# karpathy/minbpe

Hardware: AMD Instinct MI355X
Metric: BPE merges/sec (higher is better)
Workload: dtype int32; 1 GPU; regex1g: RegexTokenizer.train, 1 GB synth seed 2, vocab 32000; mode=default, parallelism=single

## Files before the change

### minbpe_amd/_native.py

```python
import ctypes as C
import os
import sys

import numpy as np

_HERE = os.path.dirname(os.path.abspath(__file__))
LIB_PATH = os.environ.get("MINBPE_AMD_LIB", os.path.join(_HERE, "lib", "libbpe_hip.so"))

BPE_OK = 0
BPE_E_HIP = -1
BPE_E_ARG = -2
BPE_E_EMPTY_STATS = -3
BPE_E_STATE = -4
BPE_E_CAP = -5
BPE_E_LIMIT = -6
BPE_E_INTERNAL = -7

PROF_KINDS = ("widen", "pair_count", "argmax", "merge", "table", "encode", "decode")

if not os.path.exists(LIB_PATH):
    raise ImportError(
        f"{LIB_PATH} is missing: build it with `python -m minbpe_amd.build` "
        "(hipcc --offload-arch=gfx950). minbpe_amd has no CPU fallback.")

# ... 387 lines not shown
                return 1

        cb = ALLREDUCE_FN(_cb)
        rc = _lib.bpe_dp_train_cb(self._h, num_merges, rank, nranks, C.cast(cb, C.c_void_p), None, _ptr(pairs),
                                  _ptr(counts), _ptr(lens), C.byref(done))
        d = done.value
        self.last_train = dict(
            pairs=list(map(tuple, pairs[:2 * d].reshape(d, 2).tolist())),
            counts=counts[:d].tolist(), lens=lens[:d].tolist(), iter_ms=None, n_done=d)
        if raised:
            raise raised[0]
        self._check(rc)
        return self.last_train

    def encode_batch(self, pairs, merge_ids, data, offsets=None):
        buf = np.frombuffer(data, dtype=np.uint8) if not isinstance(data, np.ndarray) else data
        off, n_off = self._offsets(offsets)
        n_chunks = n_off if off is not None else 1
        pm = np.ascontiguousarray(pairs, dtype=np.int32).reshape(-1)
        M = len(pm) // 2
        mi = None if merge_ids is None else np.ascontiguousarray(merge_ids, dtype=np.int32)
        out = np.empty(max(len(buf), 1), np.int32)
        oo = np.zeros(n_chunks + 1, np.uint64)
        n_out = _u64(0)
        self._check(_lib.bpe_encode_batch(self._h, _ptr(pm) if M else None, _ptr(mi), M,
                                          _ptr(buf) if len(buf) else None, len(buf), _ptr(off),
                                          n_off, _ptr(out), _ptr(oo), C.byref(n_out)))
        return out[:n_out.value], oo

    def encode_batch_resident(self, pairs, merge_ids, d_bytes: int, n: int, d_offsets: int, n_chunks: int,
                              d_ids_out: int, d_out_offsets: int) -> int:
        p = np.ascontiguousarray(pairs, dtype=np.int32).reshape(-1)
        mids = None if merge_ids is None else np.ascontiguousarray(merge_ids, dtype=np.int32)
        total = _u64(0)
        self._check(_lib.bpe_encode_batch_resident(
            self._h, _ptr(p) if len(p) else None, None if mids is None else _ptr(mids), len(p) // 2,
            C.c_void_p(d_bytes), n, C.c_void_p(d_offsets), n_chunks, C.c_void_p(d_ids_out), C.c_void_p(d_out_offsets),
            C.byref(total)))
        return int(total.value)

    def decode_set_vocab(self, blob: bytes, offsets):
        buf = np.frombuffer(blob, dtype=np.uint8)
        off = np.ascontiguousarray(offsets, dtype=np.uint64)
        self._check(_lib.bpe_decode_set_vocab(self._h, _ptr(buf) if len(buf) else None, _ptr(off),
                                              len(off) - 1))

    def decode_batch(self, ids, doc_offsets=None):
        arr = np.ascontiguousarray(ids, dtype=np.int32)
        nb, bad = _u64(0), _u64(0)
        rc = _lib.bpe_decode_batch(self._h, _ptr(arr) if len(arr) else None, len(arr), C.byref(nb),
                                   C.byref(bad))
        if rc == BPE_E_ARG and bad.value != 0xFFFFFFFFFFFFFFFF:
            raise InvalidToken(int(bad.value))
        self._check(rc)
        out = np.empty(max(nb.value, 1), np.uint8)
        if doc_offsets is None:
            self._check(_lib.bpe_decode_read(self._h, _ptr(out), len(out), None, 0, None))
            return out[:nb.value].tobytes()
        doff = np.ascontiguousarray(doc_offsets, dtype=np.uint64)
        boff = np.zeros(len(doff), np.uint64)
        self._check(_lib.bpe_decode_read(self._h, _ptr(out), len(out), _ptr(doff), len(doff), _ptr(boff)))
        return out[:nb.value].tobytes(), boff

    def decode_set_sparse(self, sparse_ids, v_dense: int):
        arr = np.ascontiguousarray(sparse_ids, dtype=np.int32)
        self._check(_lib.bpe_decode_set_sparse(self._h, _ptr(arr) if len(arr) else None, len(arr), int(v_dense)))

    def decode_batch_resident(self, d_ids: int, id_width: int, n: int, d_doc_off: int, k: int, d_out: int, out_cap: int,
                              d_boff: int) -> int:
        nb, bad = _u64(0), _u64(0)
        rc = _lib.bpe_decode_batch_resident(self._h, C.c_void_p(d_ids), id_width, n, C.c_void_p(d_doc_off), k,
                                            C.c_void_p(d_out), out_cap, C.c_void_p(d_boff), C.byref(nb), C.byref(bad))
        if rc == BPE_E_ARG and bad.value != 0xFFFFFFFFFFFFFFFF:
            raise InvalidToken(int(bad.value))
        if rc == BPE_E_CAP:
            raise OutputTooSmall(int(nb.value), (_lib.bpe_last_error(self._h) or b"").decode())
        self._check(rc)
        return int(nb.value)

    def prof_reset(self):
        self._check(_lib.bpe_prof_reset(self._h))

    def train_stats(self):
        out = np.zeros(11, np.uint64)
        self._check(_lib.bpe_train_stats_ex(self._h, _ptr(out), 11))
        return dict(dense=int(out[0]), sparse=int(out[1]), index_builds=int(out[2]), slots=int(out[3]),
                    lean=int(out[4]), deferred=int(out[5]), chained=int(out[6]), steps=int(out[7]),
                    selections=int(out[8]), slot_ids=int(out[9]), fused_steps=int(out[10]))

    def prof_read(self):
        k = len(PROF_KINDS)
        ms = np.zeros(k, np.float64)
        launches = np.zeros(k, np.uint64)
        nbytes = np.zeros(k, np.uint64)
        self._check(_lib.bpe_prof_read(self._h, _ptr(ms), _ptr(launches), _ptr(nbytes)))
        return {name: dict(ms=float(ms[i]), launches=int(launches[i]), alg_bytes=int(nbytes[i]))
                for i, name in enumerate(PROF_KINDS)}
```

### minbpe_amd/csrc/api/api_basic.hip

```cpp

extern "C" {

const char *bpe_version(void) { return "minbpe_amd libbpe_hip 0.1 (gfx950)"; }

const char *bpe_last_error(bpe_ctx *ctx) { return ctx ? ctx->err.c_str() : g_create_err.c_str(); }

int bpe_create(int device_id, bpe_ctx **out) {
    if (!out) return fail(nullptr, BPE_E_ARG, "out is NULL");
    *out = nullptr;
    int ndev = 0;
    hipError_t e = hipGetDeviceCount(&ndev);
    if (e != hipSuccess || ndev == 0)
        return fail(nullptr, BPE_E_HIP, "no HIP device available: %s",
                    e != hipSuccess ? hipGetErrorString(e) : "device count is 0");
    if (device_id < 0 || device_id >= ndev)
        return fail(nullptr, BPE_E_ARG, "device %d out of range (%d devices)", device_id, ndev);
    bpe_ctx *c = new bpe_ctx();
    c->device = device_id;
    auto bail = [&](const char *what, hipError_t er) {
        int rc = fail(nullptr, BPE_E_HIP, "%s failed: %s", what, hipGetErrorString(er));
        delete c;
        return rc;
    };
    if ((e = hipSetDevice(device_id)) != hipSuccess) return bail("hipSetDevice", e);
// ... 87 lines not shown
    } else if (!strcmp(name, "sparse")) {
        if (value < 0 || value > 2) return fail(c, BPE_E_ARG, "sparse must be 0 (never), 1 (auto) or 2 (always)");
        c->use_sparse = (int)value;
    } else if (!strcmp(name, "rep_max")) {
        if (value < 0 || value > 8) return fail(c, BPE_E_ARG, "rep_max must be 0..8");
        c->rep_max = (int)value;
    } else if (!strcmp(name, "rep_min")) {
        if (value < 0 || value > 8) return fail(c, BPE_E_ARG, "rep_min: 0..8");
        c->rep_min = value;
    } else if (!strcmp(name, "lds_delta")) {
        c->lds_delta = value != 0;
    } else if (!strcmp(name, "exp_no_delta")) {
        c->exp_no_delta = value != 0;
    } else if (!strcmp(name, "tie_window")) {
        c->tie_window = value != 0;
    } else if (!strcmp(name, "tie_index")) {
        c->tie_index = value != 0;
    } else if (!strcmp(name, "sparse_ratio")) {
        if (value < 1 || value > 64) return fail(c, BPE_E_ARG, "sparse_ratio must be 1..64");
        c->sparse_ratio = (int)value;
    } else if (!strcmp(name, "lean")) {
        if (value < 0 || value > 2) return fail(c, BPE_E_ARG, "lean must be 0 (never), 1 (auto) or 2 (always)");
        c->lean = (int)value;
    } else if (!strcmp(name, "lean_backoff")) {
        c->lean_backoff = value != 0;
    } else if (!strcmp(name, "lean_count")) {
        if (value < 0) return fail(c, BPE_E_ARG, "lean_count must be >= 0");
        c->lean_count = value;
    } else if (!strcmp(name, "lean_grid")) {
        if (value < 1 || value > 65535) return fail(c, BPE_E_ARG, "lean_grid must be 1..65535");
        c->lean_grid = (int)value;
    } else if (!strcmp(name, "enc_chain")) {
        c->enc_chain = value != 0;
    } else if (!strcmp(name, "enc_cache")) {
        c->enc_cache = value != 0;
    } else if (!strcmp(name, "enc_hash_bits")) {
        if (value < 0 || value > 40) return fail(c, BPE_E_ARG, "enc_hash_bits must be 0..40");
        c->enc_hash_bits = (int)value;
    } else if (!strcmp(name, "dec_copy")) {
        c->dec_copy = value != 0;
    } else if (!strcmp(name, "dec_window")) {
        if (value < 1024 || value > 32768 || value % 16) return fail(c, BPE_E_ARG, "dec_window: 1024..32768 bytes, a multiple of 16");
        c->dec_window = (int)value;
    } else if (!strcmp(name, "dec_tile")) {
        if (value < 256 || value > 16384 || value % 256) return fail(c, BPE_E_ARG, "dec_tile: 256..16384 tokens, a multiple of 256");
        c->dec_tile = (int)value;
    } else if (!strcmp(name, "prof_stride")) {
        if (value < 1 || value > 1024) return fail(c, BPE_E_ARG, "prof_stride must be 1..1024");
        c->prof_stride = (int)value;
    } else if (!strcmp(name, "lean_select")) {
        c->lean_select = value != 0;
    } else if (!strcmp(name, "aa_sparse")) {
        c->aa_sparse = value != 0;
    } else if (!strcmp(name, "dp_force_comm")) {
        c->dp_force_comm = value != 0;
    } else if (!strcmp(name, "dp_kcap")) {
        if (value < 1 || value > DP_KCAP_MAX) return fail(c, BPE_E_ARG, "dp_kcap must be 1..%d", DP_KCAP_MAX);
        c->dp_kcap = (int)value;
    } else if (!strcmp(name, "fuse_load")) {
        c->fuse_load = value != 0;
    } else if (!strcmp(name, "chain_dense")) {
        c->chain_dense = value != 0;
    } else if (!strcmp(name, "chain_prefetch")) {
        c->chain_prefetch = value != 0;
    } else if (!strcmp(name, "count_is_removed")) {
        c->count_is_removed = value != 0;
    } else if (!strcmp(name, "enc_long")) {
        c->enc_long = value != 0;
    } else if (!strcmp(name, "small_slots")) {
        if (value < 0 || value > 2) return fail(c, BPE_E_ARG, "small_slots: 0, 1 or 2");
        c->small_slots = (int)value;
    } else if (!strcmp(name, "chain_kcap")) {
        if (value < 1 || value > CH_KSWEEP) return fail(c, BPE_E_ARG, "chain_kcap must be 1..%d", CH_KSWEEP);
        c->chain_kcap = (int)value;
    } else if (!strcmp(name, "enc_replay")) {
        if (value < 0 || value > 1) return fail(c, BPE_E_ARG, "enc_replay must be 0 or 1");
        c->enc_replay = (int)value;
    } else if (!strcmp(name, "pinned_upload")) {
        if (value < 0 || value > 1) return fail(c, BPE_E_ARG, "pinned_upload must be 0 or 1");
        c->pinned_upload = (int)value;
    } else if (!strcmp(name, "fuse_step")) {
        if (value < 0 || value > 1) return fail(c, BPE_E_ARG, "fuse_step must be 0 or 1");
        c->fuse_step = (int)value;
    } else if (!strcmp(name, "pool_hint")) {
        if (value < 0 || value > 128) return fail(c, BPE_E_ARG, "pool_hint must be 0..128");
        c->pool_hint = (int)value;
    } else if (!strcmp(name, "chain_scan")) {
        if (value < 1 || value > 255) return fail(c, BPE_E_ARG, "chain_scan must be 1..255");
        c->chain_scan = value;
    } else if (!strcmp(name, "chain")) {
        c->chain = value != 0;
    } else if (!strcmp(name, "lean_chain")) {
        c->lean_chain = value != 0;
    } else if (!strcmp(name, "lean_sum")) {
        c->lean_sum = value != 0;
    } else if (!strcmp(name, "lean_scan")) {
        if (value < 1 || value > 1024) return fail(c, BPE_E_ARG, "lean_scan must be 1..1024");
        c->lean_scan = (int)value;
    } else if (!strcmp(name, "repack_acc")) {
        if (value < 0 || value > 10000) return fail(c, BPE_E_ARG, "repack_acc must be 0..10000");
        c->repack_acc = (int)value;
    } else if (!strcmp(name, "depth")) {
        if (value < 0 || value > 64) return fail(c, BPE_E_ARG, "depth must be 0..64");
        c->depth = (int)value;
    } else {
        return fail(c, BPE_E_ARG, "unknown option '%s'", name);
    }
    return BPE_OK;
}

static int check_offsets(bpe_ctx *c, const uint64_t *chunk_offsets, uint64_t n_chunks, uint64_t n) {
    if (!chunk_offsets) return BPE_OK;
    auto scan = [&](uint64_t lo, uint64_t hi) -> uint64_t {
        uint64_t prev = lo ? chunk_offsets[lo - 1] : 0;
        for (uint64_t i = lo; i < hi; i++) {
            const uint64_t o = chunk_offsets[i];
            if (o < prev || o > n) return i;
            prev = o;
        }
        return ~0ull;
    };
    uint64_t bad = ~0ull;
    const unsigned hw = std::max(1u, std::thread::hardware_concurrency());
    const uint64_t T = n_chunks < (1ull << 22) ? 1 : std::max<uint64_t>(1, std::min<uint64_t>(16, hw / 2));
    if (T == 1) {
        bad = scan(0, n_chunks);
    } else {
        std::vector<uint64_t> first(T, ~0ull);
        std::vector<std::thread> pool;
        const uint64_t per = (n_chunks + T - 1) / T;
        for (uint64_t w = 0; w < T; w++)
            pool.emplace_back([&, w] { first[w] = scan(std::min(n_chunks, w * per), std::min(n_chunks, (w + 1) * per)); });
        for (std::thread &t : pool) t.join();
        for (uint64_t w = 0; w < T; w++) bad = std::min(bad, first[w]);
    }
    if (bad != ~0ull)
        return fail(c, BPE_E_ARG, "chunk_offsets[%llu] = %llu: offsets must ascend and stay <= n = %llu",
                    (unsigned long long)bad, (unsigned long long)chunk_offsets[bad], (unsigned long long)n);
    return BPE_OK;
}

static int load_bytes_impl(bpe_ctx *c, const uint8_t *bytes, uint64_t n, const uint64_t *chunk_offsets,
                           uint64_t n_chunks, const uint8_t *wexp) {
    if (!c || (!bytes && n)) return fail(c, BPE_E_ARG, "bytes is NULL");
    TRY(check_offsets(c, chunk_offsets, n_chunks, n));
    if (n >= (1ull << 32)) return fail(c, BPE_E_LIMIT, "stream of %llu bytes exceeds 2^32-1 per GPU",
                                       (unsigned long long)n);
    if (wexp && !chunk_offsets) return fail(c, BPE_E_ARG, "weights need chunk offsets");
    if (wexp) {
        unsigned __int128 stands_for = 0;
        for (uint64_t i = 0; i < n_chunks; i++) {
            if (wexp[i] > 31) return fail(c, BPE_E_ARG, "weight exponent %u of chunk %llu exceeds 31", wexp[i],
                                          (unsigned long long)i);
            const uint64_t b = chunk_offsets[i], e = i + 1 < n_chunks ? chunk_offsets[i + 1] : n;
            if (e > b && e <= n) stands_for += (unsigned __int128)(e - b) << wexp[i];
        }
        if (stands_for >= ((unsigned __int128)1 << 32))
            return fail(c, BPE_E_LIMIT, "the weighted chunks stand for >= 2^32 bytes of text (32-bit pair counts)");
    }
    HIPCHK(c, hipSetDevice(c->device));
    if (n + 16 > c->cap_bytes) {
        TRY(dev_realloc(c, c->d_bytes, (size_t)n + 16));
        c->cap_bytes = n + 16;
    }
    if (n) TRY(upload_h2d(c, c->d_bytes, bytes, n));
    static const uint64_t zero = 0;
// ... 233 lines not shown
```

### minbpe_amd/csrc/api/api_ctx.hip

```cpp

struct DpComm {
    bpe_allreduce_fn fn = nullptr;
    void *user = nullptr;
    int rank = 0, nranks = 1;
};

struct bpe_ctx {
    int device = 0;
    int num_cus = 256;
    hipStream_t stream = nullptr;
    bool own_stream = false;
    std::string err;

    uint8_t *d_bytes = nullptr;
    uint64_t nbytes = 0, cap_bytes = 0;
    uint64_t *d_offsets = nullptr;
    uint64_t n_chunks = 0, cap_offsets = 0;
    bool have_bytes = false;
    uint8_t *d_wexp = nullptr;
    const struct DpComm *dp_comm = nullptr;
    long long *d_dp_ckey = nullptr;
    uint32_t *d_dp_cfold = nullptr;
    uint64_t cap_dp_cfold = 0;
    bool dp_force_comm = false;
// ... 15 lines not shown
    uint32_t vcur = 0;
    bool stats_valid = false;

    DevState *d_st = nullptr;
    uint64_t *d_tsum = nullptr, *d_tile_off = nullptr;
    uint8_t *d_tile_sin = nullptr;
    unsigned long long *d_sup = nullptr;
    uint64_t cap_tiles = 0;
    IterRec *h_rec = nullptr;
    int rec_cap = 0;
    unsigned long long *d_scratch = nullptr;
    uint32_t *d_delta = nullptr;
    uint32_t *d_dirty_list = nullptr;
    uint32_t *d_dirty_n = nullptr;
    int depth = 8;
    int repack_acc = 200;
    double repack_waste = 0.0;
    int use_slots = 2;
    int fused_rows = 0;
    uint32_t sel_epoch = 0;
    unsigned long long apply_target = 0;
    int rep_shift = 5;
    bool slotted = false;
    uint64_t slot_T = 0;
    int mq = 0;
    uint32_t *d_meta[2] = {nullptr, nullptr};
    uint4 *d_hdr[2] = {nullptr, nullptr};
    uint32_t *d_slot_lens = nullptr;
    unsigned long long *d_slot_off = nullptr, *d_slot_bsum = nullptr;
    uint32_t *d_ids2 = nullptr;
    bool slot2 = false;
    SlotHdr *d_hdr2[2] = {nullptr, nullptr};
    StageRec *d_stage = nullptr;
    uint32_t *d_smask = nullptr;
    uint32_t *d_cand = nullptr;
    uint32_t *d_idx = nullptr;
    uint32_t *d_idx_tmp = nullptr;
    uint32_t *d_idx_dirty = nullptr;
    uint32_t *d_removed = nullptr;
    uint64_t idx_cap_words = 0;
    uint64_t idx_cap_rows = 0;
    bool idx_rebuild = false;
    bool last_aa_indexed = false;
    bool idx_live = false;
    int use_sparse = 1;
    int rep_max = 8;
    int rep_min = 4;
    int lds_delta = 1;
    int exp_no_delta = 0;
    int tie_window = 0;
    int tie_index = 1;
    int sparse_ratio = 1;
    uint64_t last_count = ~0ull;
    uint64_t n_sparse = 0, n_dense = 0, n_index_builds = 0;
    uint64_t n_lean = 0, n_deferred = 0;
    int lean = 1;
    int64_t lean_count = 1 << 20;
    int lean_backoff = 1;
    int lean_grid = 256;
    int lean_scan = 31;
    int lean_select = 1;
    int aa_sparse = 1;
    int lean_chain = 1;
    int chain_dense = 1;
    unsigned long long *d_chain_req = nullptr;
    int ts = TILE2_MAX;
    int small_slots = 1;
    int count_is_removed = 1;
    int chain_prefetch = 1;
    int chain_kcap = CH_KSWEEP;
    int fuse_step = 0;
    unsigned long long *d_step_pub = nullptr;
    uint32_t *d_step_bar = nullptr;
    uint32_t step_bar_target = 0;
    bool forced = false;
    int32_t *d_forced = nullptr;
    uint64_t cap_forced = 0;
    int enc_replay = 1;
    int pinned_upload = 1;
    uint8_t *h_stage = nullptr;
    hipEvent_t ev_stage[4] = {nullptr, nullptr, nullptr, nullptr};
    bool stage_busy[4] = {false, false, false, false};
    uint64_t n_fused = 0;
    unsigned long long *d_step_stamps = nullptr;
    int pool_hint = 0;
    PoolEnt *d_pool = nullptr;
    uint32_t *d_pool_gather = nullptr;
    int chain_scan = 127;
    int chain = 1;
    StepRec *h_srec = nullptr;
    uint64_t n_steps = 0, n_full = 0, n_chained = 0;
    int lean_sum = 1;
    uint4 *d_lean_sum = nullptr;
    bool sum_valid = false;
    uint32_t *d_dbits = nullptr;
    unsigned long long *d_lean_res = nullptr;
    uint32_t lean_tag = 0;
    bool rows_pending = false;
    uint64_t cap_slots = 0;
    int dp_rank = 0, dp_nranks = 1, dp_merges = 0, dp_enq = 0, dp_done = 0;
    bool dp_active = false;
    void *comm = nullptr;
    int comm_rank = 0, comm_nranks = 1;
    uint32_t *d_dp_folded = nullptr, *d_dp_table = nullptr;
    long long *d_dp_key = nullptr;
    uint64_t dp_cur_len = 0;
    bool dp_sparse = false;
    uint32_t dp_dl = 0;
    std::vector<uint8_t> dp_flip;
    int merge_impl = 0;
    unsigned long long *d_desc = nullptr;
    unsigned long long *d_gdesc = nullptr;
    uint64_t cap_desc = 0;
    uint32_t epoch = 0;
    uint32_t lb_tune = 1;

    uint32_t *d_enc_tmp = nullptr, *d_enc_len = nullptr;
    int32_t *d_enc_out = nullptr;
    unsigned long long *d_enc_off = nullptr, *d_enc_bsum = nullptr, *d_enc_long = nullptr;
    unsigned long long *d_enc_huge = nullptr;
    int enc_long = 1;
    unsigned long long *d_ht_keys = nullptr;
    uint32_t *d_ht_vals = nullptr;
    int32_t *d_merge_ids = nullptr;
    uint64_t cap_enc_n = 0, cap_enc_chunks = 0, cap_ht = 0, cap_merge_ids = 0;
    EncEntry *d_enc_tab = nullptr;
    uint32_t *d_enc_rep = nullptr;
    uint8_t *d_enc_mid = nullptr;
    uint32_t *d_enc_midn = nullptr;
    uint64_t cap_enc_tab = 0;
    int enc_cache = 1;
    int enc_chain = 1;
    int enc_hash_bits = 0;

    uint8_t *d_dec_blob = nullptr, *d_dec_out = nullptr;
    unsigned long long *d_dec_voff = nullptr, *d_dec_off = nullptr, *d_dec_bsum = nullptr;
    int32_t *d_dec_ids = nullptr;
    uint32_t *d_dec_len = nullptr;
    uint64_t cap_dec_blob = 0, cap_dec_voff = 0, cap_dec_n = 0, cap_dec_out = 0;
    uint32_t dec_V = 0;
    bool dec_have_vocab = false, dec_have_result = false;
    uint64_t dec_n = 0, dec_total = 0;
    int32_t *d_dec_sparse = nullptr;
    uint64_t cap_dec_sparse = 0;
    uint32_t dec_V_dense = 0, dec_n_sparse = 0;
    int dec_copy = 1;
    int dec_window = 8192;
    int dec_tile = 1024;

    int mode = 1;
    int profile = 0;
    int prof_iter = -1;
    int prof_stride = 64;
    bool prof_active = false;
    int scan_sup_min = 1024;
    int k1 = 2;
    bool stream_is_bytes = false;

    std::vector<ProfEv> prof_open;
    std::vector<hipEvent_t> ev_pool;
    double prof_ms[BPE_PROF_NKINDS] = {0};
    uint64_t prof_launches[BPE_PROF_NKINDS] = {0};
    uint64_t prof_bytes[BPE_PROF_NKINDS] = {0};
};

#define GK(c, kern) ((c)->ts == TILE2_MIN ? bpe::bpe_g1::kern : bpe::bpe_g4::kern)
// ... 810 lines not shown

int launch_lean(bpe_ctx *c, uint32_t newid, int iter, IterRec *rec, bool use_index) {
    const uint32_t T = (uint32_t)c->slot_T;
    const uint32_t dl = delta_layout(c, newid);
    AbArgs A;
    A.b0 = c->d_ids[0];
    A.b1 = c->d_ids[1];
    A.hdr_in = c->d_hdr2[c->mq];
    A.hdr_out = nullptr;
    A.stage = c->d_stage;
    A.smask = c->d_smask;
    A.T = T;
    A.st = c->d_st;
    A.newid = newid;
    A.delta = c->d_delta;
    A.vcap = dl;
    A.idx = c->idx_live ? c->d_idx : nullptr;
    A.istride = (uint32_t)c->idx_cap_words;
    A.cand = nullptr;
    A.removed = c->d_removed;
    A.dirty_n = c->d_dirty_n;
    const uint32_t nwords = (T + 31) / 32;
    const unsigned g = std::max(1u, std::min(use_index ? nwords : (T + 15) / 16, (unsigned)c->lean_grid));
    TRY(prof_begin(c, BPE_PROF_MERGE, 0));
    if (c->idx_live)
        hipLaunchKernelGGL(GK(c, k_merge_ab_lean<true>), dim3(g), dim3(LEAN_MT), 0, c->stream, A, c->d_idx_dirty,
                           use_index ? 1u : 0u, c->d_dbits);
    else
        hipLaunchKernelGGL(GK(c, k_merge_ab_lean<false>), dim3(g), dim3(LEAN_MT), 0, c->stream, A, (const uint32_t *)nullptr, 0u,
                           c->d_dbits);
    LAUNCHCHK(c, "k_merge_ab_lean");
    TRY(prof_end(c));
    TRY(prof_begin(c, BPE_PROF_TABLE, 0));
    const uint32_t na = (newid + 1 + 255) / 256;
    const uint32_t ncommit = std::max(8u, std::min(128u, (nwords + 255) / 256));
    hipLaunchKernelGGL(GK(c, k_apply_lean), dim3(na + ncommit), dim3(256), 0, c->stream, c->d_mat, c->vcap, c->d_delta, dl,
                       c->d_rowmax, c->d_st, newid, c->d_dbits, c->par, rec, iter, na, c->d_hdr2[c->mq], c->d_stage,
                       c->d_removed, c->d_smask, nwords, c->d_lean_sum);
    LAUNCHCHK(c, "k_apply_lean");
    TRY(prof_end(c));
    c->par ^= 1;
    c->stats_valid = false;
    c->stream_is_bytes = false;
    c->rows_pending = true;
    c->n_lean++;
    if (use_index) c->n_sparse++; else c->n_dense++;
    return BPE_OK;
}

int launch_chain_step(bpe_ctx *c, uint32_t step, uint32_t zhi, bool use_index, bool records, bool dense = false) {
    const uint32_t T = (uint32_t)c->slot_T;
    const uint32_t dl = delta_layout(c, zhi);
    const bool fused = c->fuse_step && !c->forced && !dense && !c->dp_comm && use_index && c->idx_live;
    if (!fused) TRY(prof_begin(c, BPE_PROF_ARGMAX, 0));
    CandArgs C;
    C.idx = c->d_idx;
    C.dirty = c->d_idx_dirty;
    C.cand = nullptr;
    C.stride = (uint32_t)c->idx_cap_words;
    C.T = T;
    C.enable = 0;
    C.tie_index = 1;
    C.tie_window = 0;
    C.aa = 0;
    if (!c->idx_live) C.T = 0;
    if (dense && c->dp_comm) C.T = 0;
    (void)records;
    if (!c->d_chain_req) {
        HIPCHK(c, hipMalloc((void **)&c->d_chain_req, PL_REQ_WORDS * sizeof(unsigned long long)));
        HIPCHK(c, hipMemsetAsync(c->d_chain_req, 0, PL_REQ_WORDS * sizeof(unsigned long long), c->stream));
    }
    if (!c->d_pool) {
        HIPCHK(c, hipMalloc((void **)&c->d_pool, (3 * PL_CAP + 128) * sizeof(PoolEnt)));
        HIPCHK(c, hipMalloc((void **)&c->d_pool_gather, (2 + 2 * PL_GATHER) * sizeof(uint32_t)));
        HIPCHK(c, hipMemsetAsync(c->d_pool, 0, (3 * PL_CAP + 128) * sizeof(PoolEnt), c->stream));
        HIPCHK(c, hipMemsetAsync(c->d_pool_gather, 0, (2 + 2 * PL_GATHER) * sizeof(uint32_t), c->stream));
    }
    const DpComm *dp = c->dp_comm;
    uint32_t kcap = (uint32_t)(dense ? CH_KDENSE : std::min(CH_KSWEEP, c->chain_kcap));
    if (dp) kcap = std::min(kcap, (uint32_t)c->dp_kcap);
    if (fused) kcap = std::min(kcap, (uint32_t)STEP_KCAP);
    const uint32_t hint_below = (uint32_t)(c->pool_hint > 0 ? c->pool_hint : (int)kcap);
    const unsigned nscan = (unsigned)std::max(1, std::min(c->chain_scan, c->num_cus - 1));
    if (fused) {
        if (!c->d_step_pub) {
            HIPCHK(c, hipMalloc((void **)&c->d_step_pub, 64 * sizeof(unsigned long long)));
            HIPCHK(c, hipMemsetAsync(c->d_step_pub, 0, 64 * sizeof(unsigned long long), c->stream));
        }
        if (!c->d_step_bar) {
            HIPCHK(c, hipMalloc((void **)&c->d_step_bar, 256));
            HIPCHK(c, hipMemsetAsync(c->d_step_bar, 0, 256, c->stream));
            c->step_bar_target = 0;
        }
        const uint32_t nwords = (T + 31) / 32;
        StepArgs S;
        S.rowmax = c->d_rowmax;
        S.mat = c->d_mat;
        S.stride = c->vcap;
        S.st = c->d_st;
        S.ref = stream_ref_h(c);
        S.C = C;
        S.dbits = c->d_dbits;
        S.res = c->d_lean_res;
        S.tag = ++c->lean_tag;
        S.req = c->d_chain_req;
        S.kcap = kcap;
        S.pool = c->d_pool;
        S.gather = c->d_pool_gather;
        S.hint_below = hint_below;
        AbArgs &A = S.A;
        A.b0 = c->d_ids[0];
        A.b1 = c->d_ids[1];
        A.hdr_in = c->d_hdr2[c->mq];
        A.hdr_out = nullptr;
        A.stage = c->d_stage;
        A.smask = c->d_smask;
        A.T = T;
        A.st = c->d_st;
        A.newid = 0;
        A.delta = c->d_delta;
        A.vcap = dl;
        A.idx = c->d_idx;
        A.istride = (uint32_t)c->idx_cap_words;
        A.cand = nullptr;
        uint32_t *const removed = (c->weighted || !c->count_is_removed) ? c->d_removed : nullptr;
        A.removed = removed;
        A.dirty_n = c->d_dirty_n;
        S.idx_dirty = c->d_idx_dirty;
        S.use_index = 1u | (c->chain_prefetch ? 2u : 0u);
        const unsigned gapply = (zhi + 1 + 1023) / 1024;
        const unsigned cap = std::min((unsigned)c->num_cus, std::max(std::max((unsigned)c->lean_grid, gapply), 2u));
        const unsigned gmerge = std::max(1u, std::min(std::min(nwords, (unsigned)c->lean_grid), cap));
        const unsigned ns = std::min(nscan, cap - 1);
        const unsigned G = std::min(cap, std::max(std::max(gmerge, gapply), 1 + ns));
        if (G < gapply) return fail(c, BPE_E_INTERNAL, "fused chain step: %u workgroups cannot hold %u tokens", G, zhi + 1);
        S.nscan = ns;
        S.gm = gmerge;
        S.delta = c->d_delta;
        S.dl = dl;
        S.par = c->par;
        S.rec = c->h_rec;
        S.srec = c->h_srec;
        S.step = step;
        S.hdr_cur = c->d_hdr2[c->mq];
        S.stage = c->d_stage;
        S.removed = removed;
        S.smask = c->d_smask;
        S.nwords = nwords;
        S.sums = c->d_lean_sum;
        S.pub = c->d_step_pub;
        S.bar = c->d_step_bar;
        c->step_bar_target += G;
        S.bar_target = c->step_bar_target;
        S.stamps = c->d_step_stamps;
        TRY(prof_begin(c, BPE_PROF_MERGE, 0));
        hipLaunchKernelGGL(GK(c, k_step), dim3(G), dim3(LEAN_MT), 0, c->stream, S);
        LAUNCHCHK(c, "k_step");
        TRY(prof_end(c));
        c->par ^= 1;
        c->stats_valid = false;
        c->stream_is_bytes = false;
        c->rows_pending = true;
        c->n_steps++;
        c->n_fused++;
        c->n_sparse++;
        return BPE_OK;
    }
    if (c->forced)
        hipLaunchKernelGGL(GK(c, k_forced_sel), dim3(1), dim3(64), 0, c->stream, c->d_st, c->d_forced, c->d_mat, c->vcap, kcap);
    else
        hipLaunchKernelGGL(GK(c, k_pool_sel), dim3(1 + nscan), dim3(1024), 0, c->stream, c->d_rowmax, c->d_mat,
                           c->vcap, c->d_st, stream_ref_h(c), C, c->d_dbits, c->d_lean_res, ++c->lean_tag, c->d_chain_req,
                           kcap, c->d_pool, c->d_pool_gather, hint_below, dp ? c->d_dp_ckey : (long long *)nullptr,
                           (unsigned long long)(dp ? dp->rank : 0), c->d_pool + PL_CAP);
    LAUNCHCHK(c, "k_pool_sel");
    if (dp) {
        TRY(dp_allreduce(c, c->d_dp_ckey, DP_KEY_WORDS, BPE_DT_INT64, BPE_OP_MIN));
        hipLaunchKernelGGL(GK(c, k_pool_sel_dp), dim3(1), dim3(PL_CAP), 0, c->stream, c->d_st, c->d_dp_ckey, kcap, c->d_pool,
                           c->d_pool + PL_CAP, hint_below);
        LAUNCHCHK(c, "k_pool_sel_dp");
    }
    TRY(prof_end(c));
    AbArgs A;
    A.b0 = c->d_ids[0];
    A.b1 = c->d_ids[1];
    A.hdr_in = c->d_hdr2[c->mq];
    A.hdr_out = dense ? c->d_hdr2[c->mq ^ 1] : nullptr;
    A.stage = c->d_stage;
    A.smask = c->d_smask;
    A.T = T;
    A.st = c->d_st;
    A.newid = 0;
    A.delta = c->d_delta;
    A.vcap = dl;
    A.idx = c->idx_live ? c->d_idx : nullptr;
    A.istride = (uint32_t)c->idx_cap_words;
    A.cand = nullptr;
    uint32_t *const removed = (c->weighted || dp || !c->count_is_removed) ? c->d_removed : nullptr;
    A.removed = removed;
    A.dirty_n = c->d_dirty_n;
    const uint32_t nwords = (T + 31) / 32;
    TRY(prof_begin(c, BPE_PROF_MERGE, 0));
    if (dense) {
        const unsigned g = std::max(1u, std::min((T + 15) / 16, (unsigned)c->num_cus));
        hipLaunchKernelGGL(GK(c, k_merge_chain_dense), dim3(g), dim3(LEAN_MT), 0, c->stream, A, c->d_dbits);
        const unsigned g1 = std::max(1u, std::min((T + MT / 64 - 1) / (MT / 64), 5u * (unsigned)c->num_cus));
        hipLaunchKernelGGL(GK(c, k_merge_chain_dense1), dim3(g1), dim3(MT), 0, c->stream, A);
    } else {
        const unsigned g = std::max(1u, std::min(use_index ? nwords : (T + 15) / 16, (unsigned)c->lean_grid));
        hipLaunchKernelGGL(GK(c, k_merge_chain), dim3(g), dim3(LEAN_MT), 0, c->stream, A, c->d_idx_dirty,
                           (use_index ? 1u : 0u) | (c->chain_prefetch ? 2u : 0u), c->d_dbits);
    }
    LAUNCHCHK(c, "k_merge_chain");
    TRY(prof_end(c));
    TRY(prof_begin(c, BPE_PROF_TABLE, 0));
    const uint32_t na = (zhi + 1 + 255) / 256;
    const uint32_t ncommit = std::max(8u, std::min(128u, (nwords + 255) / 256));
    const uint32_t fS = std::min<uint32_t>(c->vcap, ((zhi + 1 + 63) / 64) * 64);
    uint32_t *ftail = dp ? c->d_dp_cfold + (size_t)2 * kcap * fS : nullptr;
    if (dp) {
        hipLaunchKernelGGL(GK(c, k_dp_fold_chain), dim3(na), dim3(256), 0, c->stream, c->d_delta, dl, c->d_st, c->d_dp_cfold, fS, ftail);
        LAUNCHCHK(c, "k_dp_fold_chain");
        TRY(dp_allreduce(c, c->d_dp_cfold, (uint64_t)2 * kcap * fS + 64, BPE_DT_INT32, BPE_OP_SUM));
    }
    hipLaunchKernelGGL(GK(c, k_apply_chain), dim3(na + ncommit), dim3(256), 0, c->stream, c->d_mat, c->vcap, c->d_delta, dl, c->d_rowmax,
                       c->d_st, c->d_dbits, c->par, c->h_rec, c->h_srec, step, na, c->d_hdr2[c->mq], c->d_stage,
                       removed, c->d_smask, nwords, c->d_lean_sum, dp ? c->d_dp_cfold : (const uint32_t *)nullptr, fS,
                       (const uint32_t *)ftail);
    LAUNCHCHK(c, "k_apply_chain");
    TRY(prof_end(c));
    c->par ^= 1;
    if (dense) c->mq ^= 1;
    c->stats_valid = false;
    c->stream_is_bytes = false;
    c->rows_pending = true;
    c->n_steps++;
    if (use_index) c->n_sparse++; else c->n_dense++;
    return BPE_OK;
}

constexpr size_t STAGE_PIECE = 32u << 20;
constexpr int STAGE_R = 4, STAGE_T_MAX = 16;
int upload_h2d(bpe_ctx *c, void *dst, const void *src, size_t bytes) {
    if (!bytes) return BPE_OK;
    if (!c->pinned_upload || bytes < 2 * STAGE_PIECE) {
        HIPCHK(c, hipMemcpyAsync(dst, src, bytes, hipMemcpyHostToDevice, c->stream));
        return BPE_OK;
    }
    if (!c->h_stage) {
        if (hipHostMalloc((void **)&c->h_stage, STAGE_PIECE * STAGE_R, hipHostMallocDefault) != hipSuccess) {
            c->h_stage = nullptr;
            (void)hipGetLastError();
            HIPCHK(c, hipMemcpyAsync(dst, src, bytes, hipMemcpyHostToDevice, c->stream));
            return BPE_OK;
        }
        for (int r = 0; r < STAGE_R; r++) HIPCHK(c, hipEventCreateWithFlags(&c->ev_stage[r], hipEventDisableTiming));
    }
    const unsigned hw = std::max(1u, std::thread::hardware_concurrency());
    const int T = (int)std::max(1u, std::min((unsigned)STAGE_T_MAX, hw / 2));
    const size_t pieces = (bytes + STAGE_PIECE - 1) / STAGE_PIECE;
    std::atomic<long long> go{-1};
    std::atomic<unsigned long long> done{0};
    const uint8_t *s8 = static_cast<const uint8_t *>(src);
    uint8_t *stage = c->h_stage;
    auto worker = [&](int w) {
        for (size_t i = 0; i < pieces; i++) {
            while (go.load(std::memory_order_acquire) < (long long)i) std::this_thread::yield();
            const size_t len = std::min(STAGE_PIECE, bytes - i * STAGE_PIECE);
            const size_t per = (len + (size_t)T - 1) / (size_t)T, lo = std::min(len, per * (size_t)w), hi = std::min(len, lo + per);
            if (hi > lo) memcpy(stage + (i % STAGE_R) * STAGE_PIECE + lo, s8 + i * STAGE_PIECE + lo, hi - lo);
            done.fetch_add(1, std::memory_order_release);
        }
    };
    std::vector<std::thread> pool;
    pool.reserve((size_t)T);
    for (int w = 1; w < T; w++) pool.emplace_back(worker, w);
    int rc = BPE_OK;
    hipError_t err = hipSuccess;
    for (size_t i = 0; i < pieces; i++) {
        if (c->stage_busy[i % STAGE_R] && err == hipSuccess) {
            err = hipEventSynchronize(c->ev_stage[i % STAGE_R]);
            c->stage_busy[i % STAGE_R] = false;
        }
        go.store((long long)i, std::memory_order_release);
        {
            const size_t len = std::min(STAGE_PIECE, bytes - i * STAGE_PIECE);
            const size_t per = (len + (size_t)T - 1) / (size_t)T, hi = std::min(len, per);
            if (hi) memcpy(stage + (i % STAGE_R) * STAGE_PIECE, s8 + i * STAGE_PIECE, hi);
            done.fetch_add(1, std::memory_order_release);
        }
        while (done.load(std::memory_order_acquire) < (unsigned long long)T * (i + 1)) std::this_thread::yield();
        if (err == hipSuccess) {
            const size_t len = std::min(STAGE_PIECE, bytes - i * STAGE_PIECE);
            err = hipMemcpyAsync(static_cast<uint8_t *>(dst) + i * STAGE_PIECE, stage + (i % STAGE_R) * STAGE_PIECE, len,
                                 hipMemcpyHostToDevice, c->stream);
            if (err == hipSuccess) err = hipEventRecord(c->ev_stage[i % STAGE_R], c->stream);
            if (err == hipSuccess) c->stage_busy[i % STAGE_R] = true;
        }
    }
    for (std::thread &t : pool) t.join();
    if (err != hipSuccess) rc = fail(c, BPE_E_HIP, "pinned upload: %s", hipGetErrorString(err));
    return rc;
}

int download_d2h(bpe_ctx *c, void *dst, const void *src_dev, size_t bytes) {
    if (!bytes) return BPE_OK;
    if (!c->pinned_upload || bytes < 2 * STAGE_PIECE || !c->h_stage) {
        HIPCHK(c, hipMemcpyAsync(dst, src_dev, bytes, hipMemcpyDeviceToHost, c->stream));
        HIPCHK(c, hipStreamSynchronize(c->stream));
        return BPE_OK;
    }
// ... 54 lines not shown
```

### minbpe_amd/csrc/api/api_prof.hip

```cpp

extern "C" {

int bpe_prof_reset(bpe_ctx *c) {
    if (!c) return BPE_E_ARG;
    TRY(prof_drain(c));
    for (int k = 0; k < BPE_PROF_NKINDS; k++) {
        c->prof_ms[k] = 0;
        c->prof_launches[k] = 0;
        c->prof_bytes[k] = 0;
    }
    return BPE_OK;
}

int bpe_prof_read(bpe_ctx *c, double *ms, uint64_t *launches, uint64_t *alg_bytes) {
    if (!c) return BPE_E_ARG;
    TRY(prof_drain(c));
    for (int k = 0; k < BPE_PROF_NKINDS; k++) {
        if (ms) ms[k] = c->prof_ms[k];
        if (launches) launches[k] = c->prof_launches[k];
        if (alg_bytes) alg_bytes[k] = c->prof_bytes[k];
    }
    return BPE_OK;
}

int bpe_train_stats(bpe_ctx *c, uint64_t *out4) {
    if (!c || !out4) return BPE_E_ARG;
    out4[0] = c->n_dense;
    out4[1] = c->n_sparse;
    out4[2] = c->n_index_builds;
    out4[3] = c->slot_T;
    return BPE_OK;
}

int bpe_train_stats_ex(bpe_ctx *c, uint64_t *out, int n) {
    if (!c || !out || n < 0) return BPE_E_ARG;
    uint64_t chained = 0;
    if (n > 6 && c->d_st) {
        DevState stt;
        TRY(read_state(c, &stt));
        chained = stt.chain_taken;
    }
    const uint64_t v[11] = {c->n_dense, c->n_sparse, c->n_index_builds, c->slot_T, c->n_lean, c->n_deferred,
                            chained + c->n_chained, c->n_steps, c->n_full, (uint64_t)c->ts, c->n_fused};
    for (int i = 0; i < n && i < 11; i++) out[i] = v[i];
    return BPE_OK;
}

}
```

### minbpe_amd/csrc/api/api_rccl.hip

```cpp

namespace {
struct RcclUid { char internal[128]; };
struct RcclApi {
    void *h = nullptr;
    int (*GetUniqueId)(RcclUid *) = nullptr;
    int (*CommInitRank)(void **, int, RcclUid, int) = nullptr;
    int (*AllReduce)(const void *, void *, size_t, int, int, void *, hipStream_t) = nullptr;
    int (*CommDestroy)(void *) = nullptr;
    int (*CommAbort)(void *) = nullptr;
    const char *(*GetErrorString)(int) = nullptr;
};
constexpr int RCCL_INT32 = 2, RCCL_INT64 = 4, RCCL_SUM = 0, RCCL_MIN = 3;

RcclApi *rccl() {
    static RcclApi api;
    static bool tried = false;
    if (!tried) {
        tried = true;
        for (const char *name : {"librccl.so.1", "librccl.so", "/opt/rocm/lib/librccl.so.1"}) {
            api.h = dlopen(name, RTLD_NOW | RTLD_LOCAL);
            if (api.h) break;
        }
        if (api.h) {
            api.GetUniqueId = (int (*)(RcclUid *))dlsym(api.h, "ncclGetUniqueId");
// ... 14 lines not shown
            return fail((c), BPE_E_HIP, "%s failed: %s", #call,                              \
                        rccl()->GetErrorString ? rccl()->GetErrorString(r_) : "rccl error"); \
    } while (0)
}

extern "C" int bpe_comm_available(void) { return rccl() ? 1 : 0; }

extern "C" int bpe_comm_unique_id(uint8_t *out128) {
    if (!out128) return BPE_E_ARG;
    RcclApi *r = rccl();
    if (!r) return fail(nullptr, BPE_E_HIP, "librccl not found");
    RcclUid id;
    if (r->GetUniqueId(&id) != 0) return fail(nullptr, BPE_E_HIP, "ncclGetUniqueId failed");
    memcpy(out128, id.internal, 128);
    return BPE_OK;
}

extern "C" int bpe_comm_init(bpe_ctx *c, int32_t rank, int32_t nranks, const uint8_t *id128) {
    if (!c || !id128 || rank < 0 || nranks < 1 || rank >= nranks) return fail(c, BPE_E_ARG, "bad arguments");
    RcclApi *r = rccl();
    if (!r) return fail(c, BPE_E_HIP, "librccl not found");
    HIPCHK(c, hipSetDevice(c->device));
    if (c->comm) {
        r->CommDestroy(c->comm);
        c->comm = nullptr;
    }
    RcclUid id;
    memcpy(id.internal, id128, 128);
    RCCLCHK(c, r->CommInitRank(&c->comm, nranks, id, rank));
    c->comm_rank = rank;
    c->comm_nranks = nranks;
    return BPE_OK;
}

extern "C" int bpe_comm_destroy(bpe_ctx *c) {
    if (!c) return BPE_E_ARG;
    if (c->comm && rccl()) {
        (void)hipSetDevice(c->device);
        (void)hipStreamSynchronize(c->stream);
        rccl()->CommDestroy(c->comm);
    }
    c->comm = nullptr;
    return BPE_OK;
}

namespace {
int dp_train_loop(bpe_ctx *c, int32_t num_merges, const DpComm &comm, int32_t *pairs_out, uint64_t *counts_out,
                  uint64_t *len_out, int32_t *n_done) {
    if (n_done) *n_done = 0;
    if (c->mode != 1 || c->use_slots != 2 || c->merge_impl != 0)
        return fail(c, BPE_E_STATE, "sharded training needs the default engine (mode 1, slots 2, merge 0)");
    struct CommScope {
        bpe_ctx *c;
        ~CommScope() { c->dp_comm = nullptr; }
    } scope{c};
    c->dp_comm = &comm;
    TRY(bpe_dp_begin(c, num_merges, comm.rank, comm.nranks));
    TRY(ensure_srec(c));
    if (!c->d_dp_ckey) HIPCHK(c, hipMalloc((void **)&c->d_dp_ckey, DP_KEY_WORDS * sizeof(long long)));
    const uint64_t cfold_words = (uint64_t)2 * DP_KCAP_MAX * c->vcap + 64;
    if (cfold_words > c->cap_dp_cfold) {
        TRY(dev_realloc(c, c->d_dp_cfold, (size_t)cfold_words));
        c->cap_dp_cfold = cfold_words;
    }
    HIPCHK(c, hipMemsetAsync(c->d_dp_cfold, 0, cfold_words * sizeof(uint32_t), c->stream));
    HIPCHK(c, hipMemsetAsync(c->d_dp_ckey, 0, DP_KEY_WORDS * sizeof(long long), c->stream));
    TRY(dp_allreduce(c, c->d_dp_table, 2 * 256 * 256, BPE_DT_INT32, BPE_OP_SUM));
    TRY(bpe_dp_table_ready(c));

    enum { U_GENERAL = 0, U_CHAIN = 2 };
    struct Unit {
        int kind, iter;
        uint32_t step;
        uint8_t hdr_flip, pass_kind;
    };
    std::deque<Unit> q;
    std::vector<long long> lens((size_t)std::max(num_merges, 1), 0);
    int done = 0, rc = BPE_OK, n_chain_inflight = 0;
    uint32_t steps = 0;
    bool stop = false, in_chain = false;
    int general_until = -1, defer_hold = 0, defer_strikes = 0;
    uint64_t lean_at_last_defer = 0, n_chain_merges = 0;
    c->n_lean = c->n_deferred = 0;
    c->n_steps = c->n_full = c->n_chained = 0;
    c->rows_pending = false;
    c->sum_valid = false;

    auto take_record = [&](int j) -> int {
        volatile IterRec *r = &c->h_rec[j];
        if (r->status == ST_EMPTY) {
            stop = true;
            rc = fail(c, BPE_E_EMPTY_STATS, "max() arg is an empty sequence (iteration %d)", j);
            return BPE_OK;
        }
        if (r->status != ST_OK) {
            stop = true;
            rc = fail(c, BPE_E_INTERNAL, "sharded training failed at iteration %d (device status %u)", j, r->status);
            return BPE_OK;
        }
        if (pairs_out) {
            pairs_out[2 * j] = r->a;
            pairs_out[2 * j + 1] = r->b;
        }
        if (counts_out) counts_out[j] = r->count;
        lens[(size_t)j] = (long long)r->new_len;
        if (c->profile) c->prof_bytes[BPE_PROF_MERGE] += 4 * (2 * c->dp_cur_len + r->new_len);
        c->dp_cur_len = r->new_len;
        c->n = r->new_len;
        c->last_count = r->count;
        if (r->a == r->b && c->idx_live && !aa_through_index(c)) c->idx_rebuild = true;
        done = j + 1;
        c->dp_done = done;
        return BPE_OK;
    };
    auto wait_iter = [&](int j) -> int {
        volatile IterRec *r = &c->h_rec[j];
        for (uint64_t spins = 1; r->seq != (unsigned long long)j + 1; spins++) {
            if ((spins & 0xFFFF) == 0 && hipStreamQuery(c->stream) == hipSuccess && r->seq != (unsigned long long)j + 1)
                return fail(c, BPE_E_INTERNAL, "iteration %d never reported (stream idle)", j);
        }
        __sync_synchronize();
        return BPE_OK;
    };
    auto wait_step = [&](uint32_t s) -> int {
        volatile StepRec *r = &c->h_srec[s % STEP_RING];
        for (uint64_t spins = 1; r->seq != (unsigned long long)s + 1; spins++) {
            if ((spins & 0xFFFF) == 0 && hipStreamQuery(c->stream) == hipSuccess && r->seq != (unsigned long long)s + 1)
                return fail(c, BPE_E_INTERNAL, "chain step %u never reported (stream idle)", s);
        }
        __sync_synchronize();
        return BPE_OK;
    };
    auto handle_deferral = [&](bool a_eq_b) -> int {
        HIPCHK(c, hipStreamSynchronize(c->stream));
        for (const Unit &u : q) {
            if (u.kind == U_CHAIN) c->n_steps--;
            if (u.pass_kind == 1) c->n_sparse--; else if (u.pass_kind == 2) c->n_dense--;
        }
        q.clear();
        n_chain_inflight = 0;
        hipLaunchKernelGGL(GK(c, k_clear_defer_chain), dim3(1), dim3(1), 0, c->stream, c->d_st);
        LAUNCHCHK(c, "k_clear_defer_chain");
        c->rows_pending = true;
        c->n_deferred++;
        if (c->lean_backoff && !a_eq_b) {
            defer_strikes = (n_chain_merges - lean_at_last_defer < 16) ? defer_strikes + 1 : 0;
            lean_at_last_defer = n_chain_merges;
            defer_hold = defer_strikes >= 2 ? std::min(32 << std::min(defer_strikes - 2, 5), 1024) : 0;
        } else if (a_eq_b) {
            defer_hold = 0;
        }
        general_until = done + 1 + defer_hold;
        in_chain = false;
        return BPE_OK;
    };

    while (!stop && done < num_merges) {
        const int lb = done + (int)q.size();
        bool enqueued = false;
        if (lb < num_merges && (int)q.size() <= c->depth) {
            const int i = lb;
            const bool want_chain = c->chain && c->lean && c->lean_select && c->tie_index && i > 0 && i >= general_until &&
                                    c->last_count != ~0ull && c->last_count <= (uint64_t)c->lean_count;
            const int hi_dense = std::min(num_merges, done + (int)q.size() * CH_KDENSE + CH_KDENSE);
            const bool want_dense = !want_chain && c->chain && c->chain_dense && c->lean && c->lds_delta && i > 0 &&
                                    i >= general_until && c->last_count != ~0ull && 256 + hi_dense + 1 <= (int)CH_DCAP;
// ... 164 lines not shown
```

### minbpe_amd/csrc/api/api_train.hip

```cpp

extern "C" {

int bpe_train(bpe_ctx *c, int32_t num_merges, int32_t *pairs_out, uint64_t *counts_out,
              double *iter_ms_out, uint64_t *len_out, int32_t *n_done) {
    if (!c || num_merges < 0) return fail(c, BPE_E_ARG, "bad arguments");
    if (!c->have_bytes) return fail(c, BPE_E_STATE, "bpe_load_bytes first");
    if (c->dp_active) return fail(c, BPE_E_STATE, "bpe_dp_end first");
    static const bool timing = getenv("BPE_TIMING") != nullptr;
    auto now = [] { return std::chrono::steady_clock::now(); };
    auto t_begin = now();
    struct ProfIterReset {
        bpe_ctx *c;
        ~ProfIterReset() { c->prof_iter = -1; }
    } prof_iter_reset{c};
    if (n_done) *n_done = 0;
    HIPCHK(c, hipSetDevice(c->device));
    TRY(ensure_table(c, 256u + (uint32_t)num_merges));
    TRY(ensure_rec(c, std::max(num_merges, 1)));
    memset(c->h_rec, 0, sizeof(IterRec) * (size_t)std::max(num_merges, 1));
    TRY(ensure_srec(c));
    const bool delta = (c->mode == 1);
    EventList ev_list;
    std::vector<hipEvent_t> &evs = ev_list.v;
    struct EvSpan {
        int ev, first, k;
    };
    std::vector<EvSpan> ev_spans;
    auto record_event = [&]() -> int {
        hipEvent_t e = nullptr;
        if (hipEventCreate(&e) != hipSuccess) return -1;
        evs.push_back(e);
        if (hipEventRecord(e, c->stream) != hipSuccess) return -1;
        return (int)evs.size() - 1;
    };
    TRY(prof_begin(c, BPE_PROF_TABLE, 0));
    HIPCHK(c, hipMemsetAsync(c->d_mat, 0, (size_t)c->vcap * c->vcap * sizeof(uint32_t), c->stream));
    HIPCHK(c, hipMemsetAsync(c->d_delta, 0, ((size_t)c->vcap * 4 * DELTA_REPL + 256 * DELTA_SKEW) * sizeof(uint32_t), c->stream));
    HIPCHK(c, hipMemsetAsync(c->d_rowmax, 0, (size_t)c->vcap * 2 * sizeof(uint32_t), c->stream));
    HIPCHK(c, hipMemsetAsync(c->d_dbits, 0, DBITS_WORDS * sizeof(uint32_t), c->stream));
    TRY(prof_end(c));
    if (iter_ms_out && record_event() < 0) return fail(c, BPE_E_HIP, "hipEventRecord failed");
    const bool fused_load = load_count_fusable(c);
    TRY(start_from_bytes(c, fused_load));
    const uint64_t n0 = c->n;
    if (!fused_load) TRY(launch_pair_count(c, false));

    int done = 0, rc = BPE_OK;
    uint64_t cur_len = n0;
    bool stop = false;
    c->rep_shift = 5;
    const bool slots = delta && c->use_slots && c->merge_impl == 0;
    const bool form2 = slots && c->use_slots == 2;
    c->idx_live = false;
    c->idx_rebuild = false;
    c->last_count = ~0ull;
    c->n_sparse = c->n_dense = c->n_index_builds = 0;
    c->n_lean = c->n_deferred = 0;
    c->n_steps = c->n_full = c->n_chained = 0;
    c->n_fused = 0;
    static const char *stamp_path = getenv("BPE_STEP_STAMPS");
    const size_t stamp_bytes = (size_t)STEP_STAMP_RING * (3 * 16 + 256 * 2) * sizeof(unsigned long long);
    if (stamp_path) {
        if (!c->d_step_stamps) HIPCHK(c, hipMalloc((void **)&c->d_step_stamps, stamp_bytes));
        HIPCHK(c, hipMemsetAsync(c->d_step_stamps, 0, stamp_bytes, c->stream));
    }
    if (c->d_step_bar) {
        HIPCHK(c, hipMemsetAsync(c->d_step_bar, 0, 256, c->stream));
        c->step_bar_target = 0;
    }
    c->rows_pending = false;
    c->sum_valid = false;
    enum { U_GENERAL = 0, U_LEAN = 1, U_CHAIN = 2 };
    struct Unit {
        int kind;
        int iter;
        uint32_t step;
        uint8_t hdr_flip;
        uint8_t aa_indexed;
        uint8_t pass_kind;
        int ev;
    };
    std::deque<Unit> q;
    int n_chain_inflight = 0;
    uint32_t steps = 0;
    int general_until = -1, defer_hold = 0, defer_strikes = 0;
    uint64_t lean_at_last_defer = 0;
    bool lean_on = false;
    bool in_chain = false;
    bool records_ok = false;
    c->ts = TILE2_MAX;
    if (slots) TRY(form2 ? slots2_enter(c) : slots_enter(c));

    int deferred = -1;
    auto take_record = [&](int j, bool aa_indexed) -> int {
        volatile IterRec *r = &c->h_rec[j];
        if (r->status == ST_DEFER) {
            deferred = j;
            return BPE_OK;
        }
        if (r->status == ST_EMPTY) {
            stop = true;
            rc = fail(c, BPE_E_EMPTY_STATS, "max() arg is an empty sequence (iteration %d)", j);
            return BPE_OK;
        }
        if (r->status != ST_OK) {
            stop = true;
            rc = fail(c, BPE_E_INTERNAL, "device status %u at iteration %d%s", r->status, j,
                      r->status == ST_LOOKBACK ? " (look-back wait timed out; set option merge=0)" : "");
            return BPE_OK;
        }
        if (pairs_out) {
            pairs_out[2 * j] = r->a;
            pairs_out[2 * j + 1] = r->b;
        }
        if (counts_out) counts_out[j] = r->count;
        if (len_out) len_out[j] = r->new_len;
        if (c->profile) {
            if (delta) {
                c->prof_bytes[BPE_PROF_MERGE] += 4 * (2 * cur_len + r->new_len);
            } else {
                c->prof_bytes[BPE_PROF_MERGE] += 4 * (cur_len + r->new_len);
                if (j > 0) c->prof_bytes[BPE_PROF_PAIR_COUNT] += 4 * cur_len;
            }
        }
        cur_len = r->new_len;
        c->n = cur_len;
        c->last_count = r->count;
        if (r->a == r->b && c->idx_live && !aa_indexed) c->idx_rebuild = true;
        c->rep_shift = 5;
        done = j + 1;
        return BPE_OK;
    };
    auto wait_iter = [&](int j) -> int {
        volatile IterRec *r = &c->h_rec[j];
        for (uint64_t spins = 1; r->seq != (unsigned long long)j + 1; spins++) {
            if ((spins & 0xFFFF) == 0 && hipStreamQuery(c->stream) == hipSuccess &&
                r->seq != (unsigned long long)j + 1)
                return fail(c, BPE_E_INTERNAL, "iteration %d never reported (stream idle)", j);
        }
        __sync_synchronize();
        return BPE_OK;
    };
// ... 97 lines not shown
                                   (lean && c->chain && c->lean_select && c->idx_live && c->tie_index && !full_rowmax);
                Unit u{U_GENERAL, i, 0u, 0, 0, 0, -1};
                if (chain) {
                    if (!chain_dense) lean_on = true;
                    if (!in_chain) {
                        TRY(flush_lean_rows(c, c->vcur));
                        hipLaunchKernelGGL(GK(c, k_set_iter), dim3(1), dim3(1), 0, c->stream, c->d_st, (uint32_t)i, (uint32_t)num_merges);
                        LAUNCHCHK(c, "k_set_iter");
                        in_chain = true;
                        records_ok = false;
                    }
                    const int hi = chain_dense ? hi_dense : std::min(num_merges, done + (int)q.size() * CH_KMAX + CH_KMAX);
                    TRY(launch_chain_step(c, steps, 255u + (uint32_t)hi, sparse, records_ok, chain_dense));
                    u.kind = U_CHAIN;
                    u.iter = -1;
                    u.step = steps++;
                    u.pass_kind = sparse ? 1 : 2;
                    u.hdr_flip = chain_dense ? 1 : 0;
                    records_ok = true;
                    n_chain_inflight++;
                    enqueued = true;
                } else if (known) {
                    in_chain = false;
                    records_ok = false;
                    if (lean && !c->forced) {
                        lean_on = true;
                        if (c->lean_select && c->lean_sum && c->sum_valid && c->idx_live && c->tie_index && !full_rowmax) {
                            TRY(launch_sel_lean(c));
                        } else if (c->lean_select && c->idx_live && c->tie_index && !full_rowmax) {
                            TRY(launch_rowsel_lean(c));
                        } else {
                            TRY(flush_lean_rows(c, c->vcur));
                            TRY(launch_select(c, full_rowmax, false));
                        }
                        TRY(launch_lean(c, 256u + (uint32_t)i, i, c->h_rec, sparse));
                        u.kind = U_LEAN;
                        u.pass_kind = sparse ? 1 : 2;
                        c->sum_valid = true;
                    } else {
                        c->sum_valid = false;
                        TRY(flush_lean_rows(c, c->vcur));
                        TRY(launch_select(c, full_rowmax, sparse));
                        if (c->slotted && c->slot2) {
                            const int mq0 = c->mq;
                            TRY(launch_merge2(c, 256u + (uint32_t)i, i, c->h_rec, sparse));
                            u.hdr_flip = (uint8_t)(c->mq != mq0);
                            u.aa_indexed = (uint8_t)c->last_aa_indexed;
                        } else if (c->slotted) {
                            TRY(launch_merge_slot(c, 256u + (uint32_t)i, i, c->h_rec));
                            u.hdr_flip = 1;
                        } else {
                            TRY(launch_merge(c, 256u + (uint32_t)i, i, c->h_rec, delta));
                        }
                    }
                    enqueued = true;
                }
                if (enqueued) {
                    if (iter_ms_out && (u.ev = record_event()) < 0) return fail(c, BPE_E_HIP, "hipEventRecord failed");
                    q.push_back(u);
                }
            }
        }
        if (!q.empty() && ((int)q.size() > c->depth || !enqueued)) {
            const Unit u = q.front();
            if (u.kind == U_CHAIN) {
                TRY(wait_step(u.step));
                const StepRec sr = *const_cast<const StepRec *>(&c->h_srec[u.step % STEP_RING]);
                if (sr.status == ST_DEFER) {
                    if ((int)sr.first_iter != done)
                        return fail(c, BPE_E_INTERNAL, "chain step %u deferred merge %u, the host expected %d", u.step, sr.first_iter, done);
                    TRY(handle_deferral((sr.pad >> 8) == 1));
                } else if (sr.status == ST_EMPTY) {
                    stop = true;
                    rc = fail(c, BPE_E_EMPTY_STATS, "max() arg is an empty sequence (iteration %d)", done);
                } else if (sr.status != ST_OK) {
                    stop = true;
                    rc = fail(c, BPE_E_INTERNAL, "device status %u at iteration %d (chain step %u)", sr.status, done, u.step);
                } else {
                    if (sr.k && (int)sr.first_iter != done)
                        return fail(c, BPE_E_INTERNAL, "chain step %u did merges from %u on, the host expected %d", u.step, sr.first_iter, done);
                    for (uint32_t j = 0; j < sr.k && !stop; j++) {
                        TRY(wait_iter((int)(sr.first_iter + j)));
                        TRY(take_record((int)(sr.first_iter + j), true));
                    }
                    if (sr.k) {
                        c->n_lean += sr.k;
                        if ((sr.pad & 0xFF) == CH_FULL) c->n_full++;
                        c->n_chained += (sr.pad & 0xFF) == CH_FULL ? sr.k - 1 : sr.k;
                        if (u.ev >= 0) ev_spans.push_back({u.ev, (int)sr.first_iter, (int)sr.k});
                    }
                    q.pop_front();
                    n_chain_inflight--;
                }
            } else {
                TRY(wait_iter(u.iter));
                TRY(take_record(u.iter, u.aa_indexed != 0));
                if (deferred >= 0) {
                    TRY(handle_deferral(c->h_rec[u.iter].a == c->h_rec[u.iter].b));
                } else if (!stop) {
                    if (u.ev >= 0) ev_spans.push_back({u.ev, u.iter, 1});
                    q.pop_front();
                }
            }
        }
        if (done >= num_merges) break;
    }
    c->prof_iter = -1;
    auto t_drain = now();
    HIPCHK(c, hipStreamSynchronize(c->stream));
    if (!stop) {
        for (const Unit &u : q) {
            if (u.kind == U_CHAIN) c->n_steps--;
            if (u.pass_kind == 1) c->n_sparse--; else if (u.pass_kind == 2) c->n_dense--;
        }
        q.clear();
        TRY(flush_lean_rows(c, 256u + (uint32_t)done));
    }
    c->rows_pending = false;
    auto t_tail = now();
    if (c->slotted) {
        if (stop) {
            const int back = (int)q.size();
            if (back & 1) c->par ^= 1;
            if (c->slot2) {
                for (const Unit &u : q)
                    if (u.hdr_flip) c->mq ^= 1;
            } else if (back & 1) {
                c->mq ^= 1;
            }
            hipLaunchKernelGGL(k_set_status, dim3(1), dim3(1), 0, c->stream, c->d_st, 0u);
        }
        TRY(c->slot2 ? slots2_leave(c) : slots_leave(c));
        HIPCHK(c, hipStreamSynchronize(c->stream));
        c->n = cur_len;
        c->vcur = 256u + (uint32_t)done;
    } else {
        c->par = done & 1;
        c->n = cur_len;
        c->vcur = 256u + (uint32_t)done;
    }
    if (iter_ms_out) {
        int prev = 0;
        for (const EvSpan &sp : ev_spans) {
            float ms = 0.f;
            HIPCHK(c, hipEventElapsedTime(&ms, evs[(size_t)prev], evs[(size_t)sp.ev]));
            for (int j = 0; j < sp.k; j++)
                if (sp.first + j < done) iter_ms_out[sp.first + j] = ms / sp.k;
            prev = sp.ev;
        }
    }
    TRY(prof_drain(c));
    if (stamp_path && c->d_step_stamps) {
        std::vector<unsigned long long> h(stamp_bytes / sizeof(unsigned long long));
        HIPCHK(c, hipMemcpy(h.data(), c->d_step_stamps, stamp_bytes, hipMemcpyDeviceToHost));
        if (FILE *f = fopen(stamp_path, "wb")) {
            fwrite(h.data(), 1, stamp_bytes, f);
            fclose(f);
        }
    }
    if (timing) {
        auto ms = [](auto a, auto b) { return std::chrono::duration<double, std::milli>(b - a).count(); };
        fprintf(stderr, "[bpe_train] %d merges: setup+enqueue of the first pass %.2f ms, loop %.2f ms, drain %.2f ms, "
                        "re-pack + timers %.2f ms\n", done, ms(t_begin, t_loop), ms(t_loop, t_drain), ms(t_drain, t_tail),
                ms(t_tail, now()));
    }
    if (n_done) *n_done = done;
// ... 5 lines not shown
```

### minbpe_amd/csrc/bpe_device.h

```cpp
#pragma once
#include <stdint.h>

namespace bpe {

constexpr uint32_t FLAG = 0x80000000u;
constexpr uint32_t IDMASK = 0x03FFFFFFu;
constexpr int WSHIFT = 26;
constexpr uint32_t WMASK = 0x7C000000u;
constexpr uint32_t NWMASK = ~WMASK;
constexpr uint32_t INVALID_WORD = 0xFFFFFFFFu;
constexpr uint32_t EMPTY_KEY = 0xFFFFFFFFu;
constexpr unsigned long long NOPOS = ~0ull;

constexpr int MT = 256;
#define BPE_GEOMETRY(NS, MJV, IDXH_LOG2)                                                                         \
    namespace NS {                                                                                               \
    constexpr int MJ = MJV;                            \
    constexpr int WAVE_SPAN = MJ * 256;                                                                          \
    constexpr int TILE = (MT / 64) * WAVE_SPAN;  \
                      \
    constexpr int TILE2 = WAVE_SPAN;                                                                             \
                                  \
    constexpr uint32_t IDX_H = 1u << IDXH_LOG2;                                                                  \
    constexpr int IDX_SHIFT = 32 - IDXH_LOG2;                                                                    \
// ... 80 lines not shown
    uint32_t status;
    int32_t tied[2 * TIE_CAP];
    int32_t fin_a, fin_b;
    unsigned long long removed;
    unsigned long long apply_done;
    uint32_t sel_tie;
    uint32_t sel_done;
    uint32_t adj;
    uint32_t ncand;
    uint32_t gap;
    uint32_t tlive;
    uint32_t defer;
    uint32_t scan_a, scan_b, scan_z;
    uint32_t chain_n, chain_pos, chain_cut;
    uint32_t chain_taken;
    uint32_t sel_ran;
    int32_t chain[2 * TIE_CAP];
    uint32_t iter;
    uint32_t num_merges;
    uint32_t sel_mode;
    uint32_t tl_n, tl_M, tl_skip;
    uint32_t bk, bz0;
    int32_t ba[CH_KMAX], bb[CH_KMAX];
    uint32_t badj[CH_KMAX];
    uint32_t bcnt[CH_KMAX];
    uint32_t brep;
    uint32_t bhm, bhm_key;
    uint32_t dp_wait;
    uint32_t pool_n, pool_theta;
    uint32_t pool_hint;
    uint32_t pool_hint_next;
    unsigned long long pool_epoch;
    alignas(128) uint32_t sel_flag;
    uint32_t pad_flag_[31];
};

struct CandArgs {
    const uint32_t *idx, *dirty;
    uint32_t *cand;
    uint32_t stride;
    uint32_t T;
    uint32_t enable;
    uint32_t tie_index;
    uint32_t tie_window;
    uint32_t aa;
};
struct AbArgs {
    uint32_t *b0, *b1;
    const SlotHdr *hdr_in;
    SlotHdr *hdr_out;
    StageRec *stage;
    uint32_t *smask;
    uint32_t T;
    DevState *st;
    uint32_t newid;
    uint32_t *delta;
    uint32_t vcap;
    uint32_t *idx;
    uint32_t istride;
    const uint32_t *cand;
    uint32_t *removed;
    uint32_t *dirty_n;
};
struct AaArgs {
    const uint32_t *b0, *b1;
    uint32_t *w0, *w1;
    const SlotHdr *hdr_in;
    SlotHdr *hdr_out;
    StageRec *stage;
    uint32_t *smask;
    uint32_t T;
    DevState *st;
    uint32_t newid;
    uint32_t *delta;
    uint32_t vcap;
    unsigned long long *sdesc;
    uint32_t epoch;
    uint32_t *dirty;
    uint32_t *removed;
    const uint32_t *cand;
    uint32_t *idx;
    uint32_t istride;
};
struct PoolEnt {
    uint32_t xy, c;
    unsigned long long key;
};

constexpr uint32_t STEP_RING = 4096;
struct StepRec {
    uint32_t first_iter, k;
    uint32_t status, pad;
    unsigned long long new_len;
    unsigned long long seq;
};

struct IterRec {
    int32_t a, b;
    uint32_t count;
    uint32_t status;
    unsigned long long new_len;
    unsigned long long seq;
};

struct StepArgs {
    uint32_t *rowmax, *mat;
    uint32_t stride;
    DevState *st;
    SlotRefH ref;
    CandArgs C;
    uint32_t *dbits;
    unsigned long long *res;
    uint32_t tag;
    unsigned long long *req;
    uint32_t kcap;
    PoolEnt *pool;
    uint32_t *gather;
    uint32_t hint_below;
    uint32_t nscan;
    AbArgs A;
    const uint32_t *idx_dirty;
    uint32_t use_index;
    uint32_t gm;
    uint32_t *delta;
    uint32_t dl;
    int par;
    IterRec *rec;
    StepRec *srec;
    uint32_t step;
    SlotHdr *hdr_cur;
    const StageRec *stage;
    uint32_t *removed;
    uint32_t *smask;
    uint32_t nwords;
    uint4 *sums;
    unsigned long long *pub;
    uint32_t *bar;
    uint32_t bar_target;
    unsigned long long *stamps;
};
constexpr uint32_t STEP_STAMP_RING = 8192;

}
```

### minbpe_amd/csrc/kernels/k_chain.hip

```cpp
#include <hip/hip_runtime.h>
#include <stdint.h>

#include "../bpe_device.h"

namespace bpe {
namespace BPE_G {

constexpr uint32_t CH_EX_CAP = 2048;

__device__ __forceinline__ int chain_match(const uint32_t *pa, const uint32_t *pb, uint32_t K, uint32_t w0, uint32_t w1) {
    const uint32_t x = w0 & IDMASK, y = w1 & NWMASK;
    int hit = -1;
    for (uint32_t p = 0; p < K; p++)
        if (x == pa[p] && y == pb[p]) hit = (int)p;
    return (w0 == INVALID_WORD) ? -1 : hit;
}

constexpr uint32_t CH_DCAP = 1024;
constexpr uint32_t CH_SD = 2 * CH_DCAP + 2;
__device__ __forceinline__ void chain_slot_load(const AbArgs &A, const uint32_t t, uint4 (&rv)[MJ], uint4 &hv) {
    const int lane = lane_id();
    const uint32_t *src = A.b0 + (size_t)t * TILE2;
#pragma unroll
    for (int j = 0; j < MJ; j++) rv[j] = *reinterpret_cast<const uint4 *>(src + j * 256 + lane * 4);
// ... 211 lines not shown
    uint32_t cm2 = 0, ct0 = 0, ct1 = 0;
    if (bcast(mb[0], 0) & 1u) cm2 = (uint32_t)(chain_match(pa, pb, K, prev2, prev1) + 1);
    const uint32_t cm1 = s ? ip : 0u;
    if (bcast(mb[MJ - 1], 63) & 0xCu) {
        ct0 = (uint32_t)(chain_match(pa, pb, K, tail[0], tail[1]) + 1);
        ct1 = (uint32_t)(chain_match(pa, pb, K, tail[1], tail[2]) + 1);
    }
#pragma unroll
    for (int j = 0; j < MJ; j++) {
        if (!__any(mb[j] != 0)) continue;
        uint32_t upm1, dn0;
        if (j > 0) upm1 = lane_last(x[(j + MJ - 1) % MJ][3]);
        else upm1 = prev1;
        if (j < MJ - 1) dn0 = lane_first(x[(j + 1) % MJ][0]);
        else dn0 = tail[0];
        uint32_t W[7];
        W[0] = (uint32_t)dpp_mov<0x138>((int)upm1, (int)x[j][3]);
        W[1] = x[j][0];
        W[2] = x[j][1];
        W[3] = x[j][2];
        W[4] = x[j][3];
        W[5] = lane_next(x[j][0], dn0);
        W[6] = lane_next(x[j][1], (j < MJ - 1) ? lane_first(x[(j + 1) % MJ][1]) : tail[1]);
        const uint32_t lo_fill = (j > 0) ? (lane_last(jc[(j + MJ - 1) % MJ]) >> 16) : (cm2 | (cm1 << 8));
        const uint32_t hi_fill = (j < MJ - 1) ? (lane_first(jc[(j + 1) % MJ]) & 0xFFFFu) : (ct0 | (ct1 << 8));
        const uint32_t lo = (uint32_t)dpp_mov<0x138>((int)lo_fill, (int)(jc[j] >> 16));
        const uint32_t hi = lane_next(jc[j] & 0xFFFFu, hi_fill);
        const unsigned long long win = (unsigned long long)lo | ((unsigned long long)jc[j] << 16) | ((unsigned long long)hi << 48);
        if (mb[j] == 0) continue;
        uint32_t todo = mb[j];
#pragma unroll
        for (int si = 0; si < 2; si++) {
            if (todo == 0) continue;
            const uint32_t k = (uint32_t)__ffs((int)todo) - 1u;
            todo &= todo - 1u;
            const int q = j * 256 + lane * 4 + (int)k;
            const unsigned long long wk = win >> (8u * k);
            const uint32_t p = ((uint32_t)(wk >> 16) & 255u) - 1u;
            const int li = (int)((uint32_t)wk & 255u) - 1, ri = (int)((uint32_t)(wk >> 32) & 255u) - 1;
            const uint32_t Z = z0 + p;
            uint32_t *dl, *dr;
            if (DENSE) {
                dl = sd + p * CH_SD;
                dr = dl + CH_DCAP;
                atomicAdd(&dl[2 * CH_DCAP + 1], 1u);
            } else {
                if (A.removed) atomicAdd(&A.removed[(p * (uint32_t)CH_RMV + (t & (uint32_t)(CH_RMV - 1))) * REMOVED_STRIDE], 1u);
                dl = A.delta + delta_rep_off(p * (uint32_t)CH_RSTRIDE + (t & (brep - 1u)), vc);
                dr = dl + vc;
            }
            const bool k1 = (k & 1u) != 0, k2 = (k & 2u) != 0;
            const uint32_t wa = k2 ? (k1 ? W[4] : W[3]) : (k1 ? W[2] : W[1]);
            const uint32_t wt = word_weight(wa);
            const uint32_t Lw = k2 ? (k1 ? W[3] : W[2]) : (k1 ? W[1] : W[0]);
            if (!(wa & FLAG) && Lw != INVALID_WORD) {
                if (li != (int)p) {
                    const uint32_t Lseq = (li >= 0 && (uint32_t)li < p) ? z0 + (uint32_t)li : (Lw & IDMASK);
                    atomicAdd(&dl[Lseq], wt);
                    if (!DENSE || A.idx) {
                        const uint32_t Lfin = li >= 0 ? z0 + (uint32_t)li : (Lw & IDMASK);
                        index_add(A.idx, A.istride, t, Lfin, Z);
                        if (q == 0) index_add(A.idx, A.istride, tprev, Lfin, Z);
                    }
                }
            }
            const uint32_t R = k2 ? (k1 ? W[6] : W[5]) : (k1 ? W[4] : W[3]);
            if (!(R & FLAG)) {
                if (ri == (int)p) {
                    if (DENSE) atomicAdd(&dl[2 * CH_DCAP], wt);
                    else atomicAdd(&A.st->badj[p], wt);
                } else {
                    atomicAdd(&dr[(ri >= 0 && (uint32_t)ri < p) ? z0 + (uint32_t)ri : (R & IDMASK)], wt);
                }
                if (!DENSE || A.idx) {
                    const uint32_t y = ri >= 0 ? z0 + (uint32_t)ri : (R & IDMASK);
                    index_add(A.idx, A.istride, t, Z, y);
                    if (q + 2 >= (int)len) index_add(A.idx, A.istride, tnext, Z, y);
                }
            }
        }
    }
}

__device__ __forceinline__ uint32_t chain_hash_find(const uint32_t *pa, uint32_t K, uint32_t *tab) {
    if (K < 5) return 0u;
    const uint32_t lane = (uint32_t)lane_id(), half = lane >> 5, l = lane & 31u;
    const bool in = l < K;
    const uint32_t a = in ? pa[l] : 0u;
    volatile uint32_t *t = tab + half * 256u;
    for (uint32_t m = 129u; m < 256u; m += 4u) {
        const uint32_t h = (__umul24(a, m + 2u * half) >> 8) & 255u;
        if (in) t[h] = l;
        __builtin_amdgcn_fence(__ATOMIC_RELEASE, "wavefront");
        __builtin_amdgcn_wave_barrier();
        __builtin_amdgcn_fence(__ATOMIC_ACQUIRE, "wavefront");
        const bool clash = in && t[h] != l;
        const unsigned long long cb = __ballot(clash);
        if ((uint32_t)cb == 0u) return m;
        if ((uint32_t)(cb >> 32) == 0u) return m + 2u;
    }
    return 0u;
}
__device__ __forceinline__ uint32_t chain_hash_build(uint32_t *s_ph, uint32_t *s_hm, uint32_t *s_hs, const uint32_t *s_pa, uint32_t K,
                                                     bool pre_ok = false, uint32_t pre_hm = 0) {
    if (threadIdx.x < 256) s_ph[threadIdx.x] = 0xFFFFFFFFu;
    uint32_t hm = pre_hm;
    if (!pre_ok) {
        if (threadIdx.x == 0) *s_hm = 0;
        __syncthreads();
        if (wave_id() == 0) {
            const uint32_t f = chain_hash_find(s_pa, K, s_hs);
            if (lane_id() == 0) *s_hm = f;
        }
        __syncthreads();
        hm = *s_hm;
    } else {
        __syncthreads();
    }
    if (hm && threadIdx.x < K) s_ph[(__umul24(s_pa[threadIdx.x], hm) >> 8) & 255u] = (s_pa[threadIdx.x] << 8) | (threadIdx.x + 1u);
    __syncthreads();
    return hm;
}

struct MergeLds {
    alignas(16) uint32_t s_out[LEAN_MT / 64][TILE2];
    uint32_t s_list[LEAN_SUB * 32];
    uint32_t s_tot[2];
    uint32_t s_pa[CH_KMAX], s_pb[CH_KMAX], s_pb1[CH_KMAX + 1];
    uint32_t s_ph[256], s_hm;
    uint32_t s_hs[512];
};
template <bool THROUGH = false>
__device__ __forceinline__ void merge_chain_body(const AbArgs &A, const uint32_t *__restrict__ idx_dirty, uint32_t use_index,
                                                 MergeLds &L, const uint32_t K, const uint32_t z0, const uint32_t brep,
                                                 const uint32_t blk, const uint32_t nblk, unsigned long long *dbg = nullptr,
                                                 const bool have_st = false, const uint32_t tlive_in = 0, const uint32_t gap_in = 0,
                                                 const bool pre_ok = false, const uint32_t pre_hm = 0) {
    auto dstamp = [&](int i) {
        if (dbg && threadIdx.x == 0) dbg[i] = wall_clock64();
    };
    DevState *st = A.st;
    auto &s_out = L.s_out;
    auto &s_list = L.s_list;
    auto &s_tot = L.s_tot;
    auto &s_pa = L.s_pa;
    auto &s_pb = L.s_pb;
    auto &s_pb1 = L.s_pb1;
    const uint32_t hm = chain_hash_build(L.s_ph, &L.s_hm, L.s_hs, s_pa, K, pre_ok, pre_hm);
    const uint32_t *s_ph = L.s_ph;
    const uint32_t Tl = min(A.T, have_st ? tlive_in : st->tlive);
    const uint32_t gap = have_st ? gap_in : st->gap;
    constexpr uint32_t NWV = LEAN_MT / 64;
    AbArgs A1 = A;
    A1.newid = z0;
    const uint32_t a0 = s_pa[0], b0 = s_pb[0];
    auto do_slot = [&](uint32_t t) {
        if (K == 1) {
            merge_ab_wave<true, true, false, THROUGH>(s_out[wave_id()], nullptr, t, A1, a0, b0, Tl);
        } else {
            uint4 rv[MJ], hv;
            chain_slot_load(A, t, rv, hv);
            merge_chain_wave<false, THROUGH>(s_out[wave_id()], nullptr, t, A, s_pa, s_pb, s_pb1, K, z0, brep, rv, hv, s_ph, hm, Tl);
        }
    };
    if (!(use_index & 1u) || gap != 0) {
        const uint32_t nw = nblk * NWV;
        for (uint32_t t = blk * NWV + wave_id(); t < Tl; t += nw) do_slot(t);
        return;
    }
    dstamp(8);
    const uint32_t nwords = (Tl + 31) / 32;
    const uint32_t per = (nwords + nblk - 1) / nblk;
    const uint32_t wlo = blk * per, whi = min(nwords, wlo + per);
    for (uint32_t sub = wlo; sub < whi; sub += LEAN_SUB) {
        uint32_t mk = 0;
        const uint32_t w = sub + threadIdx.x;
        if (threadIdx.x < LEAN_SUB && w < whi) {
            mk = idx_dirty[w];
            for (uint32_t p = 0; p < K; p++) {
                uint32_t h1, h2, h3;
                pair_hash(s_pa[p], s_pb[p], h1, h2, h3);
                mk |= A.idx[(size_t)h1 * A.istride + w] & A.idx[(size_t)h2 * A.istride + w] &
                      A.idx[(size_t)h3 * A.istride + w];
            }
            const uint32_t left = Tl - w * 32;
            if (left < 32) mk &= (1u << left) - 1u;
        }
        const uint32_t c = (uint32_t)__popc(mk);
        const uint32_t inc = wave_iscan_add(c);
        if (threadIdx.x < 128 && lane_id() == 63) s_tot[wave_id()] = inc;
        __syncthreads();
        const uint32_t n = s_tot[0] + s_tot[1];
        if (threadIdx.x < LEAN_SUB) {
            uint32_t o = inc - c + (wave_id() == 1 ? s_tot[0] : 0u);
            while (mk) {
                s_list[o++] = w * 32 + (uint32_t)__ffs((int)mk) - 1u;
                mk &= mk - 1u;
            }
        }
        __syncthreads();
        if (sub == wlo) dstamp(9);
        if (K == 1 || MJ > 1 || !(use_index & 2u)) {
            for (uint32_t i = wave_id(); i < n; i += NWV) do_slot(s_list[i]);
        } else {
            uint32_t i = wave_id();
            uint4 rv[MJ], hv, nrv[MJ], nhv;
            if (i < n) chain_slot_load(A, s_list[i], rv, hv);
            for (; i < n; i += NWV) {
                const bool more = i + NWV < n;
                if (more) chain_slot_load(A, s_list[i + NWV], nrv, nhv);
                merge_chain_wave<false, THROUGH>(s_out[wave_id()], nullptr, s_list[i], A, s_pa, s_pb, s_pb1, K, z0, brep, rv, hv, s_ph, hm, Tl);
                if (more) {
#pragma unroll
                    for (int j = 0; j < MJ; j++) rv[j] = nrv[j];
                    hv = nhv;
                }
            }
        }
        __syncthreads();
    }
}
enum { SW_BB = CH_KMAX, SW_BADJ = 2 * CH_KMAX, SW_BK = 3 * CH_KMAX, SW_BZ0, SW_BREP, SW_STATUS, SW_DEFER, SW_SEL_RAN, SW_TLIVE, SW_GAP, SW_BHM, SW_BHM_KEY, SW_ADJ, SW_N };
constexpr int SW_WORDS = 128;
static_assert(SW_N <= SW_WORDS, "two waves fetch the state words");
__device__ __forceinline__ void step_words_fetch(const DevState *st, uint32_t *s_w) {
    const uint32_t i = threadIdx.x;
    if (i < (uint32_t)SW_N) {
        const uint32_t *base = reinterpret_cast<const uint32_t *>(st);
        uint32_t off;
        if (i < (uint32_t)SW_BB) off = (uint32_t)offsetof(DevState, ba) / 4 + i;
        else if (i < (uint32_t)SW_BADJ) off = (uint32_t)offsetof(DevState, bb) / 4 + (i - (uint32_t)SW_BB);
        else if (i < (uint32_t)SW_BK) off = (uint32_t)offsetof(DevState, badj) / 4 + (i - (uint32_t)SW_BADJ);
        else {
            constexpr uint32_t o[SW_N - SW_BK] = {
                (uint32_t)offsetof(DevState, bk) / 4,      (uint32_t)offsetof(DevState, bz0) / 4,     (uint32_t)offsetof(DevState, brep) / 4,
                (uint32_t)offsetof(DevState, status) / 4,  (uint32_t)offsetof(DevState, defer) / 4,   (uint32_t)offsetof(DevState, sel_ran) / 4,
                (uint32_t)offsetof(DevState, tlive) / 4,   (uint32_t)offsetof(DevState, gap) / 4,     (uint32_t)offsetof(DevState, bhm) / 4,
                (uint32_t)offsetof(DevState, bhm_key) / 4, (uint32_t)offsetof(DevState, adj) / 4};
            off = o[0];
#pragma unroll
            for (int k = 1; k < SW_N - SW_BK; k++) off = (i == (uint32_t)SW_BK + (uint32_t)k) ? o[k] : off;
        }
        s_w[i] = base[off];
    }
    __syncthreads();
}
__global__ void __launch_bounds__(LEAN_MT)
k_merge_chain(AbArgs A, const uint32_t *__restrict__ idx_dirty, uint32_t use_index, uint32_t *__restrict__ dbits) {
    __shared__ MergeLds L;
    __shared__ uint32_t s_w[SW_WORDS];
    DevState *st = A.st;
    step_words_fetch(st, s_w);
    const uint32_t ran = s_w[SW_SEL_RAN];
    if (blockIdx.x == 0 && ran) {
        for (uint32_t i = threadIdx.x; i < DBITS_WORDS; i += LEAN_MT) dbits[i] = 0;
        __syncthreads();
        if (threadIdx.x == 0) st->sel_ran = 0;
    }
    const uint32_t K = s_w[SW_BK];
    if (s_w[SW_STATUS] || s_w[SW_DEFER] || K == 0) return;
    const uint32_t z0 = s_w[SW_BZ0], brep = s_w[SW_BREP];
    if (threadIdx.x < CH_KMAX) {
        L.s_pa[threadIdx.x] = threadIdx.x < K ? s_w[threadIdx.x] : 0xFFFFFFFFu;
        L.s_pb[threadIdx.x] = threadIdx.x < K ? s_w[SW_BB + threadIdx.x] : 0xFFFFFFFFu;
        L.s_pb1[threadIdx.x + 1] = threadIdx.x < K ? s_w[SW_BB + threadIdx.x] : 0xFFFFFFFFu;
        if (threadIdx.x == 0) L.s_pb1[0] = 0xFFFFFFFFu;
    }
    __syncthreads();
    merge_chain_body(A, idx_dirty, use_index, L, K, z0, brep, blockIdx.x, gridDim.x, nullptr, true, s_w[SW_TLIVE], s_w[SW_GAP],
                     s_w[SW_BHM_KEY] == ((z0 << 8) | K), s_w[SW_BHM]);
}

constexpr int CH_KDENSE = 6;
static_assert((LEAN_MT / 64) * TILE2 * 4 + CH_KDENSE * (int)CH_SD * 4 + 256 <= 160 * 1024, "dense chain pass: LDS");
__global__ void __launch_bounds__(LEAN_MT)
k_merge_chain_dense(AbArgs A, uint32_t *__restrict__ dbits) {
    __shared__ __attribute__((aligned(16))) uint32_t s_out[LEAN_MT / 64][TILE2];
    __shared__ uint32_t s_sd[CH_KDENSE * CH_SD];
    __shared__ uint32_t s_pa[CH_KMAX], s_pb[CH_KMAX], s_pb1[CH_KMAX + 1];
    DevState *st = A.st;
    const uint32_t ran = st->sel_ran;
    if (blockIdx.x == 0 && ran) {
        for (uint32_t i = threadIdx.x; i < DBITS_WORDS; i += LEAN_MT) dbits[i] = 0;
        __syncthreads();
        if (threadIdx.x == 0) st->sel_ran = 0;
    }
    const uint32_t K = st->bk;
    if (!(st->status || st->defer) && K == 1) return;
    if (st->status || st->defer || K == 0 || K > (uint32_t)CH_KDENSE) {
        const uint4 *hi = reinterpret_cast<const uint4 *>(A.hdr_in);
        uint4 *ho = reinterpret_cast<uint4 *>(A.hdr_out);
        for (size_t i = (size_t)blockIdx.x * LEAN_MT + threadIdx.x; i < 2 * (size_t)A.T; i += (size_t)gridDim.x * LEAN_MT) ho[i] = hi[i];
        if (K > (uint32_t)CH_KDENSE && blockIdx.x == 0 && threadIdx.x == 0) st->status = ST_INTERNAL;
        return;
    }
    const uint32_t z0 = st->bz0, brep = st->brep;
    if (threadIdx.x < CH_KMAX) {
        s_pa[threadIdx.x] = threadIdx.x < K ? (uint32_t)st->ba[threadIdx.x] : 0xFFFFFFFFu;
        s_pb[threadIdx.x] = threadIdx.x < K ? (uint32_t)st->bb[threadIdx.x] : 0xFFFFFFFFu;
        s_pb1[threadIdx.x + 1] = threadIdx.x < K ? (uint32_t)st->bb[threadIdx.x] : 0xFFFFFFFFu;
        if (threadIdx.x == 0) s_pb1[0] = 0xFFFFFFFFu;
    }
    for (uint32_t i = threadIdx.x; i < K * CH_SD; i += LEAN_MT) s_sd[i] = 0;
    __syncthreads();
    constexpr uint32_t NWV = LEAN_MT / 64;
    const uint32_t nw = gridDim.x * NWV;
    const uint32_t Tl = min(A.T, st->tlive);
    for (uint32_t t = blockIdx.x * NWV + wave_id(); t < A.T; t += nw)
    {
        uint4 rv[MJ], hv;
        chain_slot_load(A, t, rv, hv);
        merge_chain_wave<true>(s_out[wave_id()], s_sd, t, A, s_pa, s_pb, s_pb1, K, z0, (uint32_t)CH_RSTRIDE, rv, hv, nullptr, 0, Tl);
    }
    __syncthreads();
    const uint32_t vc = A.vcap & 0xFFFFFFu;
    const uint32_t lim = min(vc, (uint32_t)CH_DCAP);
    for (uint32_t p = 0; p < K; p++) {
        const uint32_t *sd = s_sd + p * CH_SD;
        uint32_t *g = A.delta + delta_rep_off(p * (uint32_t)CH_RSTRIDE + (blockIdx.x & (brep - 1u)), vc);
        for (uint32_t i = threadIdx.x; i < lim; i += LEAN_MT) {
            const uint32_t l = sd[i], r = sd[CH_DCAP + i];
            if (l) atomicAdd(&g[i], l);
            if (r) atomicAdd(&g[vc + i], r);
        }
        if (threadIdx.x == 0) {
            const uint32_t adj = sd[2 * CH_DCAP], rem = sd[2 * CH_DCAP + 1];
            if (adj) atomicAdd(&st->badj[p], adj);
            if (rem && A.removed) atomicAdd(&A.removed[(p * (uint32_t)CH_RMV + (blockIdx.x & (uint32_t)(CH_RMV - 1))) * REMOVED_STRIDE], rem);
        }
    }
}
__global__ void __launch_bounds__(MT, 5)
k_merge_chain_dense1(AbArgs A) {
    __shared__ __attribute__((aligned(16))) uint32_t s_out[MT / 64][TILE2];
    __shared__ uint32_t s_delta[2 * LDSD_CAP + 2];
    const DevState *st = A.st;
    if (st->status || st->defer || st->bk != 1) return;
    const uint32_t a = (uint32_t)st->ba[0], b = (uint32_t)st->bb[0];
    A.newid = st->bz0;
    ldsd_clear(s_delta);
    const uint32_t nw = gridDim.x * (MT / 64);
    const uint32_t Tl = min(A.T, st->tlive);
    for (uint32_t t = blockIdx.x * (MT / 64) + wave_id(); t < A.T; t += nw)
        merge_ab_wave<false, false, true>(s_out[wave_id()], s_delta, t, A, a, b, Tl);
    ldsd_flush(s_delta, A);
}

template <bool OWNED>
__device__ __forceinline__ void apply_chain_tokens(const uint32_t t, uint32_t *__restrict__ mat, uint32_t stride,
                                                   uint32_t *__restrict__ delta, uint32_t vcap, const uint32_t *__restrict__ rowmax,
                                                   uint32_t *__restrict__ dbits, uint4 *__restrict__ sums,
                                                   const uint32_t *__restrict__ folded, uint32_t fS, const uint32_t *__restrict__ ftail,
                                                   const uint32_t K, const uint32_t z0, const uint32_t ran,
                                                   const uint32_t *pairs, const uint32_t *adjs, const uint32_t brep_in) {
    auto dld = [&](const uint32_t *p) -> uint32_t { return OWNED ? ld_agent(p) : *p; };
    auto pair_a = [&](uint32_t p) -> uint32_t { return pairs[p] >> 16; };
    auto pair_b = [&](uint32_t p) -> uint32_t { return pairs[p] & 0xFFFFu; };
    {
        const uint32_t Zlast = z0 + K - 1u;
        if ((t & ~255u) > Zlast) return;
        const bool live = t <= Zlast;
        const uint32_t nrep = 1u << (vcap >> 24);
        const uint32_t vc = vcap & 0xFFFFFFu;
        uint2 rm = make_uint2(0u, 0u);
        uint32_t prevflag = 0, oldword = 0;
        if (OWNED) {
            oldword = ran ? 0u : dbits[t >> 5];
            prevflag = (oldword >> (t & 31)) & 1u;
            if (live) {
                const unsigned long long v = ld_agent64(reinterpret_cast<const unsigned long long *>(rowmax) + t);
                rm = make_uint2((uint32_t)v, (uint32_t)(v >> 32));
            }
        } else if (live) {
            prevflag = (dbits[t >> 5] >> (t & 31)) & 1u;
            rm = reinterpret_cast<const uint2 *>(rowmax)[t];
        }
        bool flagged = false;
        if (K == 1) {
            const uint32_t a = pair_a(0), b = pair_b(0), Z = z0;
            const uint32_t adj = folded ? ftail[0] : adjs[0];
            constexpr int RB = OWNED ? 8 : 16;
            uint32_t x[RB][2];
            auto load_batch = [&](uint32_t r0) {
#pragma unroll
                for (int k = 0; k < RB; k++) {
                    const uint32_t r = r0 + k;
                    x[k][0] = (live && r < nrep) ? dld(&delta[delta_rep_off(r, vc) + t]) : 0u;
                    x[k][1] = (live && r < nrep) ? dld(&delta[delta_rep_off(r, vc) + vc + t]) : 0u;
                }
            };
            if (!folded) load_batch(0);
            const uint32_t old_ta = live ? mat[(size_t)t * stride + a] : 0u;
            uint32_t sl = 0, sr = 0;
            if (folded) {
                sl = live ? folded[t] : 0u;
                sr = live ? folded[(size_t)fS + t] : 0u;
            }
            for (uint32_t r0 = 0; !folded;) {
#pragma unroll
                for (int k = 0; k < RB; k++) {
                    if (x[k][0]) delta[delta_rep_off(r0 + k, vc) + t] = 0;
                    if (x[k][1]) delta[delta_rep_off(r0 + k, vc) + vc + t] = 0;
                    sl += x[k][0];
                    sr += x[k][1];
                }
                r0 += RB;
                if (r0 >= nrep) break;
                load_batch(r0);
            }
            const uint32_t dr = sr + (t == a ? adj : 0u), ir = sr + (t == Z ? adj : 0u);
            if (sl) {
                atomicSub(&mat[(size_t)t * stride + a], sl);
                atomicAdd(&mat[(size_t)t * stride + Z], sl);
                flagged |= old_ta == rm.x;
            }
            if (dr) atomicSub(&mat[(size_t)b * stride + t], dr);
            if (ir) atomicAdd(&mat[(size_t)Z * stride + t], ir);
            if (live && t == b) mat[(size_t)a * stride + b] = 0;
            flagged |= live && ((t == a) | (t == b) | (t == Z));
        } else {
            const uint32_t brep = folded ? 0u : brep_in;
            constexpr int G = OWNED ? 4 : 8;
            for (uint32_t g = 0; g < K; g += G) {
                uint32_t x[G][CH_REP][2];
                if (brep == (uint32_t)CH_REP) {
#pragma unroll
                    for (int q = 0; q < G; q++) {
#pragma unroll
                        for (int r = 0; r < CH_REP; r++) {
                            const size_t o = delta_rep_off((g + (uint32_t)q) * (uint32_t)CH_RSTRIDE + (uint32_t)r, vc);
                            x[q][r][0] = (live && g + (uint32_t)q < K) ? dld(&delta[o + t]) : 0u;
                            x[q][r][1] = (live && g + (uint32_t)q < K) ? dld(&delta[o + vc + t]) : 0u;
                        }
                    }
                }
#pragma unroll
                for (int q = 0; q < G; q++) {
                    const uint32_t p = g + (uint32_t)q;
                    if (p >= K) break;
                    const uint32_t a = pair_a(p), b = pair_b(p), Z = z0 + p;
                    const uint32_t adj = folded ? ftail[p] : adjs[p];
                    uint32_t sl = 0, sr = 0;
                    if (folded) {
                        sl = live ? folded[(size_t)(2 * p) * fS + t] : 0u;
                        sr = live ? folded[(size_t)(2 * p + 1) * fS + t] : 0u;
                    } else if (brep == (uint32_t)CH_REP) {
#pragma unroll
                        for (int r = 0; r < CH_REP; r++) {
                            const size_t o = delta_rep_off(p * (uint32_t)CH_RSTRIDE + (uint32_t)r, vc);
                            if (x[q][r][0]) delta[o + t] = 0;
                            if (x[q][r][1]) delta[o + vc + t] = 0;
                            sl += x[q][r][0];
                            sr += x[q][r][1];
                        }
                    } else {
                        constexpr int YB = OWNED ? CH_RSTRIDE / 2 : CH_RSTRIDE;
#pragma unroll
                        for (int r0 = 0; r0 < CH_RSTRIDE; r0 += YB) {
                            uint32_t y[YB][2];
#pragma unroll
                            for (int r = 0; r < YB; r++) {
                                const size_t o = delta_rep_off(p * (uint32_t)CH_RSTRIDE + (uint32_t)(r0 + r), vc);
                                y[r][0] = live ? dld(&delta[o + t]) : 0u;
                                y[r][1] = live ? dld(&delta[o + vc + t]) : 0u;
                            }
#pragma unroll
                            for (int r = 0; r < YB; r++) {
                                const size_t o = delta_rep_off(p * (uint32_t)CH_RSTRIDE + (uint32_t)(r0 + r), vc);
                                if (y[r][0]) delta[o + t] = 0;
                                if (y[r][1]) delta[o + vc + t] = 0;
                                sl += y[r][0];
                                sr += y[r][1];
                            }
                        }
                    }
                    const uint32_t dr = sr + (t == a ? adj : 0u), ir = sr + (t == Z ? adj : 0u);
                    if (sl) {
                        const uint32_t old = atomicSub(&mat[(size_t)t * stride + a], sl);
                        atomicAdd(&mat[(size_t)t * stride + Z], sl);
                        flagged |= old == rm.x;
                    }
                    if (dr) atomicSub(&mat[(size_t)b * stride + t], dr);
                    if (ir) atomicAdd(&mat[(size_t)Z * stride + t], ir);
                    if (live && t == b) mat[(size_t)a * stride + b] = 0;
                    flagged |= live && ((t == a) | (t == b) | (t == Z));
                }
            }
        }
        if (OWNED) {
            const unsigned long long fb = __ballot(flagged);
            const uint32_t mine = (lane_id() < 32) ? (uint32_t)fb : (uint32_t)(fb >> 32);
            const uint32_t neww = oldword | mine;
            if ((lane_id() & 31) == 0 && (ran || neww != oldword)) dbits[t >> 5] = neww;
        } else if (flagged && !prevflag) {
            atomicOr(&dbits[t >> 5], 1u << (t & 31));
        }
        const uint32_t vs = (!live || flagged || prevflag) ? 0u : rm.x;
        const uint32_t gw = t >> 6, base = gw * 64u;
        const int lane = lane_id();
        const uint32_t m = wave_umax_dpp(vs);
        const unsigned long long bal = __ballot(m != 0 && vs == m);
        const int fl = bal ? __ffsll((long long)bal) - 1 : 0;
        const uint32_t arg = (uint32_t)__shfl((int)rm.y, fl);
        if (lane == 0) sums[gw] = make_uint4(m, base + (uint32_t)fl, arg, (uint32_t)__popcll(bal));
    }
}
__device__ __forceinline__ void apply_chain_records(DevState *st, int par, IterRec *rec, StepRec *srec, uint32_t step,
                                                    uint32_t *__restrict__ removed, const uint32_t K, const bool noop,
                                                    const uint32_t status, const uint32_t defer, const uint32_t remote) {
    {
        uint32_t v = 0;
        if (removed) {
#pragma unroll
            for (int i = 0; i < 4; i++) {
                const uint32_t x = ld_agent(&removed[(threadIdx.x * 4 + i) * REMOVED_STRIDE]);
                if (x) removed[(threadIdx.x * 4 + i) * REMOVED_STRIDE] = 0;
                v += x;
            }
        }
        static_assert(CH_RMV == 8 && 2 * CH_KMAX == 64, "lanes 2p, 2p + 1 hold the removals of pair p");
        const uint32_t tot = wave_sum_u32(v);
        v += (uint32_t)__shfl_xor((int)v, 1);
        __shared__ uint32_t rem[CH_KMAX];
        if (!(threadIdx.x & 1u)) {
            const uint32_t p = threadIdx.x >> 1;
            rem[p] = removed ? ((K == 1 && p == 0) ? tot : v) : st->bcnt[p];
        }
        __builtin_amdgcn_fence(__ATOMIC_RELEASE, "wavefront");
        __builtin_amdgcn_wave_barrier();
        __builtin_amdgcn_fence(__ATOMIC_ACQUIRE, "wavefront");
        if (threadIdx.x == 0) {
            const unsigned long long n = st->n[par];
            unsigned long long nn = n;
            const uint32_t iter = st->iter;
            const uint32_t mode_used = st->sel_mode;
            uint32_t k_done = 0;
            if (!noop) {
                for (uint32_t p = 0; p < K; p++) {
                    nn -= rem[p];
                    iter_rec_put(rec + iter + p, st->ba[p], st->bb[p], st->bcnt[p], ST_OK, nn);
                }
                k_done = K;
                st->iter = iter + K;
                st->sel_mode = (st->tl_n > st->tl_skip) ? CH_LIST : CH_FULL;
            } else if (status == 0 && !defer) {
                st->sel_mode = CH_FULL;
            }
            if (status == 0) st->n[par ^ 1] = nn;
            if (remote && st->status == 0) st->status = ST_INTERNAL;
            st->removed = 0;
            st->pool_hint = st->pool_hint_next;
            StepRec *sr = srec + (step % STEP_RING);
            step_rec_put(sr, iter, k_done, (status == 0 && defer) ? (uint32_t)ST_DEFER : status, mode_used | (defer << 8), nn);
            __builtin_amdgcn_s_waitcnt(0);
            for (uint32_t p = 0; p < k_done; p++) iter_rec_seal(rec + iter + p, (unsigned long long)(iter + p) + 1);
            step_rec_seal(sr, (unsigned long long)step + 1);
        }
    }
}
template <bool THROUGH = false>
__device__ __forceinline__ void apply_chain_commit(uint32_t first, uint32_t stp, uint32_t nwords, uint32_t *__restrict__ smask,
                                                   const StageRec *__restrict__ stage, SlotHdr *__restrict__ hdr_cur) {
    for (uint32_t w = first; w < nwords; w += stp) {
        uint32_t m = THROUGH ? ld_agent(&smask[w]) : smask[w];
        if (!m) continue;
        smask[w] = 0;
        while (m) {
            uint32_t tt[4], h[4][8];
#pragma unroll
            for (int i = 0; i < 4; i++) {
                tt[i] = m ? w * 32 + (uint32_t)__ffs((int)m) - 1u : 0xFFFFFFFFu;
                m &= m - 1u;
                if (tt[i] != 0xFFFFFFFFu) stage_get<THROUGH>(stage + tt[i], h[i]);
            }
#pragma unroll
            for (int i = 0; i < 4; i++) {
                if (tt[i] == 0xFFFFFFFFu) continue;
                uint4 *dst = reinterpret_cast<uint4 *>(hdr_cur + tt[i]);
                dst[0] = make_uint4(h[i][0], h[i][1], h[i][2], h[i][3]);
                dst[1] = make_uint4(h[i][4], h[i][5], h[i][6], h[i][7]);
            }
        }
    }
}
__global__ void __launch_bounds__(256)
k_apply_chain(uint32_t *__restrict__ mat, uint32_t stride, uint32_t *__restrict__ delta, uint32_t vcap,
              const uint32_t *__restrict__ rowmax, DevState *st, uint32_t *__restrict__ dbits, int par, IterRec *rec,
              StepRec *srec, uint32_t step, uint32_t na, SlotHdr *__restrict__ hdr_cur, const StageRec *__restrict__ stage,
              uint32_t *__restrict__ removed, uint32_t *__restrict__ smask, uint32_t nwords, uint4 *__restrict__ sums,
              const uint32_t *__restrict__ folded, uint32_t fS, const uint32_t *__restrict__ ftail) {
    __shared__ uint32_t s_w[SW_WORDS], s_pairs[CH_KMAX];
    step_words_fetch(st, s_w);
    const uint32_t remote = (folded && ftail[16] != 0) ? 1u : 0u;
    const uint32_t status = s_w[SW_STATUS] ? s_w[SW_STATUS] : (remote ? ST_INTERNAL : 0u), defer = s_w[SW_DEFER];
    const uint32_t K = s_w[SW_BK], z0 = s_w[SW_BZ0];
    const bool noop = status || defer || K == 0;
    if (blockIdx.x < na) {
        if (noop) return;
        if (threadIdx.x < CH_KMAX) s_pairs[threadIdx.x] = (s_w[threadIdx.x] << 16) | (s_w[SW_BB + threadIdx.x] & 0xFFFFu);
        if (threadIdx.x == 0 && K == 1) s_w[SW_BADJ] = s_w[SW_ADJ];
        __syncthreads();
        apply_chain_tokens<false>(blockIdx.x * 256u + threadIdx.x, mat, stride, delta, vcap, rowmax, dbits, sums, folded, fS,
                                  ftail, K, z0, 0u, s_pairs, s_w + SW_BADJ, s_w[SW_BREP]);
        return;
    }
    if (blockIdx.x == na && threadIdx.x < 64) apply_chain_records(st, par, rec, srec, step, removed, K, noop, status, defer, remote);
    if (noop) return;
    apply_chain_commit((blockIdx.x - na) * blockDim.x + threadIdx.x, (gridDim.x - na) * blockDim.x, nwords, smask, stage, hdr_cur);
}

__global__ void __launch_bounds__(256)
k_dp_fold_chain(uint32_t *__restrict__ delta, uint32_t dl, const DevState *__restrict__ st, uint32_t *__restrict__ folded,
                uint32_t S, uint32_t *__restrict__ tail) {
    const uint32_t status = st->status, K = st->bk, z0 = st->bz0;
    const bool noop = status || st->defer || K == 0;
    const uint32_t t = blockIdx.x * 256u + threadIdx.x;
    if (t < 32) tail[t] = t == 16 ? (status ? 1u : 0u) : ((!noop && t < K && t < 16) ? (K == 1 ? st->adj : st->badj[t]) : 0u);
#ifdef BPE_DP_DEBUG
    if (t >= 32 && t < 64) {
        uint32_t v = 0;
        if (t == 32) v = st->iter;
        else if (t == 33) v = st->sel_mode;
        else if (t == 34) v = K;
        else if (t == 35) v = st->tl_n;
        else if (t == 36) v = st->tl_M;
        else if (t == 37) v = st->tl_skip;
        else if (t == 38) v = st->defer;
        else if (t == 39) v = st->gap;
        else if (t < 48) v = (uint32_t)st->ba[t - 40] << 16 | (uint32_t)st->bb[t - 40];
        else v = (uint32_t)st->chain[2 * (t - 48)] << 16 | (uint32_t)st->chain[2 * (t - 48) + 1];
        tail[t] = v;
    }
#endif
    if (noop || t > z0 + K - 1u || t >= S) return;
    const uint32_t nrep = 1u << (dl >> 24), vc = dl & 0xFFFFFFu;
    if (K == 1) {
        uint32_t sl = 0, sr = 0;
        for (uint32_t r = 0; r < nrep; r++) {
            const size_t o = delta_rep_off(r, vc);
            const uint32_t x = delta[o + t], y = delta[o + vc + t];
            if (x) delta[o + t] = 0;
            if (y) delta[o + vc + t] = 0;
            sl += x;
            sr += y;
        }
        folded[t] = sl;
        folded[(size_t)S + t] = sr;
        return;
    }
    const uint32_t brep = st->brep;
    for (uint32_t p = 0; p < K; p++) {
        uint32_t x[CH_RSTRIDE][2];
#pragma unroll
        for (int r = 0; r < CH_RSTRIDE; r++) {
            const size_t o = delta_rep_off(p * (uint32_t)CH_RSTRIDE + (uint32_t)r, vc);
            x[r][0] = (uint32_t)r < brep ? delta[o + t] : 0u;
            x[r][1] = (uint32_t)r < brep ? delta[o + vc + t] : 0u;
        }
        uint32_t sl = 0, sr = 0;
#pragma unroll
        for (int r = 0; r < CH_RSTRIDE; r++) {
            const size_t o = delta_rep_off(p * (uint32_t)CH_RSTRIDE + (uint32_t)r, vc);
            if (x[r][0]) delta[o + t] = 0;
            if (x[r][1]) delta[o + vc + t] = 0;
            sl += x[r][0];
            sr += x[r][1];
        }
        folded[(size_t)(2 * p) * S + t] = sl;
        folded[(size_t)(2 * p + 1) * S + t] = sr;
    }
}
__global__ void k_dp_after_sum(DevState *st, const uint32_t *__restrict__ tail) {
    if (tail[8] != 0 && st->status == 0) st->status = ST_INTERNAL;
}

__global__ void __launch_bounds__(64)
k_forced_sel(DevState *st, const int32_t *__restrict__ pairs, const uint32_t *__restrict__ mat, uint32_t stride, uint32_t kcap) {
    const uint32_t lane = threadIdx.x;
    const uint32_t status = st->status, defer = st->defer, iter = st->iter, nm = st->num_merges;
    if (status || defer) return;
    if (iter >= nm) {
        if (lane == 0) st->bk = 0;
        return;
    }
    const uint32_t r = iter + lane;
    const bool in = lane < kcap && r < nm;
    const uint32_t a = in ? (uint32_t)pairs[2 * r] : 0xFFFFFFFEu, b = in ? (uint32_t)pairs[2 * r + 1] : 0xFFFFFFFDu;
    uint32_t bad = in ? ((a == b) | (a >= 256u + iter) | (b >= 256u + iter)) : 1u;
#pragma unroll
// ... 87 lines not shown
```

### minbpe_amd/csrc/kernels/k_merge.hip

```cpp
#include <hip/hip_runtime.h>
#include <stdint.h>

#include "../bpe_device.h"

namespace bpe {
namespace BPE_G {


struct Tile {
    uint32_t x[MJ][4];
    uint32_t rb[MJ];
    int E[MJ];
    uint32_t tail[3];
};

__device__ __forceinline__ void tile_fetch(Tile &t, const uint32_t *__restrict__ ids, uint64_t n,
                                           uint64_t tile_base) {
    const int lane = lane_id(), wave = wave_id();
    const uint64_t wbase = tile_base + (uint64_t)wave * WAVE_SPAN;
#pragma unroll
    for (int j = 0; j < MJ; j++) {
        const uint64_t p0 = wbase + j * 256 + lane * 4;
        const uint4 v = *reinterpret_cast<const uint4 *>(ids + p0);
        t.x[j][0] = (p0 + 0 < n) ? v.x : INVALID_WORD;
        t.x[j][1] = (p0 + 1 < n) ? v.y : INVALID_WORD;
        t.x[j][2] = (p0 + 2 < n) ? v.z : INVALID_WORD;
        t.x[j][3] = (p0 + 3 < n) ? v.w : INVALID_WORD;
    }
    const uint64_t tailp = wbase + WAVE_SPAN;
#pragma unroll
    for (int i = 0; i < 3; i++) t.tail[i] = (tailp + i < n) ? ids[tailp + i] : INVALID_WORD;
}

struct SlotRaw {
    uint4 v[MJ];
    uint32_t tail[3];
};
__device__ __forceinline__ void slot_raw_load(SlotRaw &r, const uint32_t *__restrict__ src, int len) {
    const int lane = lane_id(), wrel = wave_id() * WAVE_SPAN;
#pragma unroll
    for (int j = 0; j < MJ; j++) {
        const int q0 = wrel + j * 256 + lane * 4;
        r.v[j] = make_uint4(0, 0, 0, 0);
        if (q0 < len) r.v[j] = *reinterpret_cast<const uint4 *>(src + q0);
    }
#pragma unroll
    for (int i = 0; i < 3; i++) {
        const int q = wrel + WAVE_SPAN + i;
        r.tail[i] = (q < len) ? src[q] : 0u;
    }
}
__device__ __forceinline__ void tile_from_slot(Tile &t, const SlotRaw &r, int len, const uint32_t *halo) {
    const int lane = lane_id(), wrel = wave_id() * WAVE_SPAN;
#pragma unroll
    for (int j = 0; j < MJ; j++) {
        const int q0 = wrel + j * 256 + lane * 4;
        const uint32_t w[4] = {r.v[j].x, r.v[j].y, r.v[j].z, r.v[j].w};
#pragma unroll
        for (int k = 0; k < 4; k++) {
            const int q = q0 + k;
            t.x[j][k] = (q < len) ? w[k] : ((q < len + 3) ? halo[q - len] : INVALID_WORD);
        }
    }
#pragma unroll
    for (int i = 0; i < 3; i++) {
        const int q = wrel + WAVE_SPAN + i;
        t.tail[i] = (q < len) ? r.tail[i] : ((q < len + 3) ? halo[q - len] : INVALID_WORD);
    }
}

__device__ __forceinline__ void tile_rbits(Tile &t, uint32_t a, uint32_t b) {
    uint32_t nx[MJ];
    const uint32_t tail = t.tail[0];
#pragma unroll
    for (int j = 0; j < MJ; j++) {
        const uint32_t up = (j < MJ - 1) ? lane_first(t.x[(j + 1) % MJ][0]) : tail;
        nx[j] = lane_next(t.x[j][0], up);
    }
#pragma unroll
    for (int j = 0; j < MJ; j++) {
        uint32_t rb = 0;
#pragma unroll
        for (int k = 0; k < 4; k++) {
            const uint32_t nxt = (k < 3) ? t.x[j][k + 1] : nx[j];
            rb |= (uint32_t)(((t.x[j][k] & IDMASK) == a) & ((nxt & NWMASK) == b)) << k;
        }
        t.rb[j] = rb;
    }
}
__device__ __forceinline__ void tile_lzscan(Tile &t, int *s_wave) {
    const int lane = lane_id(), wave = wave_id();
    int lzg[MJ];
    const int gb0 = wave * WAVE_SPAN + lane * 4;
#pragma unroll
    for (int j = 0; j < MJ; j++) {
        const uint32_t z = (~t.rb[j]) & 0xFu;
        lzg[j] = z ? (gb0 + j * 256 + (31 - __clz((int)z))) : -1;
    }
    int carry = -1;
#pragma unroll
    for (int j = 0; j < MJ; j++) {
        const int v = wave_iscan_max(lzg[j]);
        const int ex = dpp_mov<0x138>(-1, v);
        t.E[j] = max(carry, ex);
        carry = max(carry, (int)lane_last((uint32_t)v));
    }
    if (lane == 0) s_wave[wave] = carry;
    __syncthreads();
    int win = -1;
    for (int w = 0; w < wave; w++) win = max(win, s_wave[w]);
#pragma unroll
    for (int j = 0; j < MJ; j++) t.E[j] = max(t.E[j], win);
}
__device__ __forceinline__ void tile_prepare(Tile &t, uint32_t a, uint32_t b, int *s_wave) {
    tile_rbits(t, a, b);
    tile_lzscan(t, s_wave);
}

__device__ __forceinline__ void tile_load(Tile &t, const uint32_t *__restrict__ ids, uint64_t n,
                                          uint64_t tile_base, uint32_t a, uint32_t b, int *s_wave) {
    tile_fetch(t, ids, n, tile_base);
    tile_prepare(t, a, b, s_wave);
}

__device__ __forceinline__ uint32_t parity_bit(int q, int lz, uint32_t s) {
    return (uint32_t)((q - lz) & 1) ^ ((lz < 0) ? s : 0u);
}

__device__ __forceinline__ uint32_t group_mbits(const Tile &t, int j, uint32_t s, uint32_t &mprev) {
    const int q0 = wave_id() * WAVE_SPAN + j * 256 + lane_id() * 4;
    int lz = t.E[j];
    mprev = (q0 == 0) ? s : ((lz == q0 - 1) ? 0u : parity_bit(q0 - 1, lz, s));
    uint32_t mb = 0;
#pragma unroll
    for (int k = 0; k < 4; k++) {
        if ((t.rb[j] >> k) & 1u) {
            mb |= parity_bit(q0 + k, lz, s) << k;
        } else {
            lz = q0 + k;
        }
    }
    return mb;
}

struct SummaryLds {
    uint32_t cnt[MT / 64];
    int fz[MT / 64];
    uint32_t o0;
    unsigned long long packed;
};
__device__ __forceinline__ uint64_t tile_summary(const Tile &t, int len, SummaryLds &L) {
    if (threadIdx.x == 0) L.o0 = 0;
    __syncthreads();
    uint32_t cnt = 0;
    int fz = 0x7fffffff;
    const int gb0 = wave_id() * WAVE_SPAN + lane_id() * 4;
#pragma unroll
    for (int j = 0; j < MJ; j++) {
        uint32_t mprev;
        const uint32_t mb = group_mbits(t, j, 0u, mprev);
        cnt += __popc(mb);
        const uint32_t z = (~t.rb[j]) & 0xFu;
        if (z) fz = min(fz, gb0 + j * 256 + (__ffs((int)z) - 1));
        const int q0 = gb0 + j * 256;
        if (len - 1 >= q0 && len - 1 < q0 + 4) L.o0 = (mb >> (len - 1 - q0)) & 1u;
    }
    cnt = wave_sum_u32(cnt);
    fz = wave_min_i32(fz);
    if (lane_id() == 0) {
        L.cnt[wave_id()] = cnt;
        L.fz[wave_id()] = fz;
    }
    __syncthreads();
    if (threadIdx.x == 0) {
        uint32_t M0 = 0;
        int F = 0x7fffffff;
        for (int w = 0; w < MT / 64; w++) {
            M0 += L.cnt[w];
            F = min(F, L.fz[w]);
        }
        const int P = min(F, len);
        L.packed = (uint64_t)M0 | ((uint64_t)(P & 1) << 32) | ((uint64_t)(F >= len) << 33) |
                   ((uint64_t)L.o0 << 34);
    }
    __syncthreads();
    return L.packed;
}

__global__ void __launch_bounds__(MT)
k_merge_count(const uint32_t *__restrict__ ids, const DevState *__restrict__ st, int par,
              uint64_t *__restrict__ tsum) {
    __shared__ int s_wave[MT / 64];
    __shared__ SummaryLds s_sum;
    if (st->status) return;
    const uint64_t n = st->n[par];
    const uint64_t tile_base = (uint64_t)blockIdx.x * TILE;
    if (tile_base >= n) return;
    const int len = (int)min((uint64_t)TILE, n - tile_base);
    uint32_t a, b;
    if (!resolved_pair(st, ids, a, b)) return;
    Tile t;
    tile_load(t, ids, n, tile_base, a, b, s_wave);
    const uint64_t w = tile_summary(t, len, s_sum);
    if (threadIdx.x == 0) tsum[blockIdx.x] = w;
}

struct TS {
    unsigned long long k0, k1;
    uint32_t o;
};
__device__ __forceinline__ TS ts_then(const TS &A, const TS &B) {
    const uint32_t a0 = A.o & 1u, a1 = (A.o >> 1) & 1u, b0 = B.o & 1u, b1 = (B.o >> 1) & 1u;
    TS r;
// ... 162 lines not shown
    __shared__ uint32_t s_status;
    if (threadIdx.x == 0) {
        if (dirty_n) *dirty_n = 0;
        if (st->status == 0 && !st->found) {
            uint32_t a, b;
            if (resolved_pair(st, ids, a, b)) {
                st->a = (int32_t)a;
                st->b = (int32_t)b;
                st->found = 1;
            } else {
                st->status = ST_INTERNAL;
            }
        }
        st->fin_a = st->a;
        st->fin_b = st->b;
        s_status = st->status;
        if (rec) {
            rec[iter].a = st->a;
            rec[iter].b = st->b;
            rec[iter].count = st->count;
            rec[iter].status = st->status;
        }
    }
    __syncthreads();
    if (s_status) {
        if (threadIdx.x == 0 && rec) {
            rec[iter].new_len = st->n[par];
            __threadfence_system();
            rec[iter].seq = (unsigned long long)iter + 1;
        }
        return;
    }
    const uint64_t R = (nsup + 1023) / 1024;
    const uint64_t t0 = min((uint64_t)threadIdx.x * R, nsup), t1 = min(t0 + R, nsup);
    TS mine = ts_identity();
    for (uint64_t t = t0; t < t1; t++) mine = ts_then(mine, ssum[t]);
    const int lane = lane_id(), wave = wave_id();
    TS inc = mine;
#pragma unroll
    for (int d = 1; d < 64; d <<= 1) {
        const TS p = ts_shfl_up(inc, d);
        if (lane >= d) inc = ts_then(p, inc);
    }
    if (lane == 63) s_w[wave] = inc;
    __syncthreads();
    TS pre = ts_identity();
    for (int w = 0; w < wave; w++) pre = ts_then(pre, s_w[w]);
    TS exl = ts_shfl_up(inc, 1);
    if (lane == 0) exl = ts_identity();
    pre = ts_then(pre, exl);
    if (threadIdx.x == 1023) {
        const TS all = ts_then(pre, mine);
        st->n[par ^ 1] = all.k0;
        if (rec) {
            rec[iter].new_len = all.k0;
            __threadfence_system();
            rec[iter].seq = (unsigned long long)iter + 1;
        }
    }
    for (uint64_t t = t0; t < t1; t++) {
        spre[t] = pre;
        pre = ts_then(pre, ssum[t]);
    }
}
__global__ void __launch_bounds__(SUP_TILES)
k_tile_expand(const uint64_t *__restrict__ tsum, uint64_t ntiles, const DevState *__restrict__ st, int par,
              const TS *__restrict__ spre, uint64_t *__restrict__ tile_off, uint8_t *__restrict__ tile_sin) {
    __shared__ TS s_w[SUP_TILES / 64];
    if (st->status) return;
    const uint64_t n = st->n[par];
    const uint64_t t = (uint64_t)blockIdx.x * SUP_TILES + threadIdx.x;
    const bool live = t < ntiles && t * TILE < n;
    TS mine = ts_identity();
    if (live) mine = ts_of_tile(tsum[t], (uint32_t)min((uint64_t)TILE, n - t * TILE));
    TS inc, exc;
    ts_scan_256(mine, s_w, inc, exc);
    if (live) {
        const TS pre = ts_then(spre[blockIdx.x], exc);
        tile_off[t] = pre.k0;
        tile_sin[t] = (uint8_t)(pre.o & 1u);
    }
}

template <bool DELTA, bool SKIP_UNCHANGED, int HL = 0>
__device__ __forceinline__ void tile_rewrite(const Tile &t, uint32_t s, uint32_t a, uint32_t b,
                                             uint32_t newid, uint32_t *__restrict__ dst_tile,
                                             uint32_t *s_wsum, uint32_t *__restrict__ delta,
                                             uint32_t vcap, int own_len, uint32_t *kept_out,
                                             bool *changed_out, uint32_t *__restrict__ hdr4 = nullptr,
                                             uint32_t *__restrict__ idx = nullptr, uint32_t istride = 0,
                                             uint32_t tself = 0, uint32_t tnext = 0xFFFFFFFFu) {
    const int lane = lane_id(), wave = wave_id();
    uint32_t mb[MJ], mp[MJ], kb[MJ], ex[MJ];
    uint32_t carry = 0, chg = 0;
    const int qw = wave * WAVE_SPAN + lane * 4;
#pragma unroll
    for (int j = 0; j < MJ; j++) {
        mb[j] = group_mbits(t, j, s, mp[j]);
        uint32_t valid = 0;
#pragma unroll
        for (int k = 0; k < 4; k++) valid |= (uint32_t)(qw + j * 256 + k < own_len) << k;
        chg |= mb[j] & valid;
        kb[j] = (~((mb[j] << 1) | mp[j])) & valid & 0xFu;
        const uint32_t v = wave_iscan_add((uint32_t)__popc(kb[j]));
        ex[j] = carry + v - __popc(kb[j]);
        carry += lane_last(v);
    }
    const bool wchg = __any(chg != 0);
    if (lane == 0) s_wsum[wave] = carry | (wchg ? 0x80000000u : 0u);
    __syncthreads();
    uint32_t wbase = 0, total = 0;
    bool changed = (s != 0);
    for (int w = 0; w < MT / 64; w++) {
        const uint32_t v = s_wsum[w];
        if (w < wave) wbase += v & 0x7FFFFFFFu;
        total += v & 0x7FFFFFFFu;
        changed |= (v >> 31) != 0;
    }
    if (kept_out) *kept_out = total;
    if (changed_out) *changed_out = changed;
    if (!SKIP_UNCHANGED || changed) {
        uint32_t *dst = dst_tile + wbase;
#pragma unroll
        for (int j = 0; j < MJ; j++) {
            uint32_t o = ex[j];
#pragma unroll
            for (int k = 0; k < 4; k++) {
                if ((kb[j] >> k) & 1u) {
                    const uint32_t w = t.x[j][k];
                    dst[o++] = ((mb[j] >> k) & 1u) ? (newid | (w & (FLAG | WMASK))) : w;
                }
            }
        }
        if (hdr4) {
#pragma unroll
            for (int j = 0; j < MJ; j++) {
                const uint32_t lo = wbase + ex[j], hi = lo + __popc(kb[j]);
                if (kb[j] && (lo < 3 || (HL == 0 ? hi == total : hi + 1 >= total))) {
                    uint32_t gi = lo;
#pragma unroll
                    for (int k = 0; k < 4; k++) {
                        if ((kb[j] >> k) & 1u) {
                            const uint32_t w = t.x[j][k];
                            const uint32_t ow = ((mb[j] >> k) & 1u) ? (newid | (w & (FLAG | WMASK))) : w;
                            if (gi < 3) hdr4[gi] = ow;
                            if (HL == 0) {
                                if (gi + 1 == total) hdr4[3] = ow;
                            } else {
                                if (gi + 1 == total) hdr4[5] = ow;
                                if (gi + 2 == total) hdr4[4] = ow;
                            }
                            gi++;
                        }
                    }
                }
            }
        }
    }
    if (DELTA) {
        const uint32_t t0 = t.tail[0], t1 = t.tail[1], t2 = t.tail[2];
        uint32_t near = 0;
#pragma unroll
        for (int j = 0; j < MJ; j++) near |= mb[j] | mp[j];
        near |= (uint32_t)((((t0 & IDMASK) == a) & ((t1 & NWMASK) == b)) |
                           (((t1 & IDMASK) == a) & ((t2 & NWMASK) == b)));
        if (!__any(near != 0)) return;
        const uint32_t nrep = 1u << (vcap >> 24);
        vcap &= 0xFFFFFFu;
        delta += delta_rep_off(blockIdx.x & (nrep - 1), vcap);
#pragma unroll
        for (int j = 0; j < MJ; j++) {
            const uint32_t nb_m = lane_next(mb[j], 0);
            const uint32_t nb_x0 = lane_next(t.x[j][0], 0);
            const uint32_t nb_x1 = lane_next(t.x[j][1], 0);
            uint32_t up_m, up_x0, up_x1;
            if (j < MJ - 1) {
                up_m = lane_first(mb[(j + 1) % MJ]);
                up_x0 = lane_first(t.x[(j + 1) % MJ][0]);
                up_x1 = lane_first(t.x[(j + 1) % MJ][1]);
            } else {
                const uint32_t m3 = (mb[j] >> 3) & 1u;
                const uint32_t r4 = (uint32_t)(((t0 & IDMASK) == a) & ((t1 & NWMASK) == b));
                const uint32_t m4 = r4 & (m3 ^ 1u);
                const uint32_t r5 = (uint32_t)(((t1 & IDMASK) == a) & ((t2 & NWMASK) == b));
                const uint32_t m5 = r5 & (m4 ^ 1u);
                up_m = m4 | (m5 << 1);
                up_x0 = t0;
                up_x1 = t1;
            }
            const bool last = (lane == 63);
            const uint32_t X[6] = {t.x[j][0], t.x[j][1], t.x[j][2], t.x[j][3],
                                   last ? up_x0 : nb_x0, last ? up_x1 : nb_x1};
            const uint32_t Mx = mp[j] | (mb[j] << 1) | (((last ? up_m : nb_m) & 3u) << 5);
            if (mb[j] | mp[j] | (Mx >> 5)) {
#pragma unroll
                for (int k = 0; k < 4; k++) {
                    const uint32_t Mk = (Mx >> (k + 1)) & 1u, Mkm1 = (Mx >> k) & 1u,
                                   Mkp1 = (Mx >> (k + 2)) & 1u;
                    if (qw + j * 256 + k >= own_len) continue;
                    const uint32_t wt = word_weight(X[k]);
                    if (!(X[k + 1] & FLAG) && !Mk) {
                        if (Mkm1) atomicAdd(&delta[1 * (size_t)vcap + (X[k + 1] & IDMASK)], wt);
                        else if (Mkp1) atomicAdd(&delta[0 * (size_t)vcap + (X[k] & IDMASK)], wt);
                    }
                    if (!Mkm1) {
                        const uint32_t Xq = Mk ? X[k + 2] : X[k + 1];
                        const uint32_t Mq = Mk ? ((Mx >> (k + 3)) & 1u) : Mkp1;
                        if (!(Xq & FLAG)) {
                            const int qpos = qw + j * 256 + k;
                            if (Mk) {
                                const uint32_t y = Mq ? newid : (Xq & IDMASK);
                                atomicAdd(&delta[3 * (size_t)vcap + y], wt);
                                if (idx) {
                                    index_add(idx, istride, tself, newid, y);
                                    if (qpos + 2 >= own_len && tnext != 0xFFFFFFFFu) index_add(idx, istride, tnext, newid, y);
                                }
                            } else if (Mq) {
                                atomicAdd(&delta[2 * (size_t)vcap + (X[k] & IDMASK)], wt);
                                if (idx) {
                                    index_add(idx, istride, tself, X[k] & IDMASK, newid);
                                    if (qpos + 1 >= own_len && tnext != 0xFFFFFFFFu) index_add(idx, istride, tnext, X[k] & IDMASK, newid);
                                }
                            }
                        }
                    }
                }
            }
        }
    }
}

template <bool DELTA>
__global__ void __launch_bounds__(MT)
k_merge_scatter(const uint32_t *__restrict__ in, uint32_t *__restrict__ out,
                const DevState *__restrict__ st, int par, const uint64_t *__restrict__ tile_off,
                const uint8_t *__restrict__ tile_sin, uint32_t newid, uint32_t *__restrict__ delta,
                uint32_t vcap) {
    __shared__ int s_wave[MT / 64];
    __shared__ uint32_t s_wsum[MT / 64];
    if (st->status) return;
    const uint64_t n = st->n[par];
    const uint64_t tile_base = (uint64_t)blockIdx.x * TILE;
    if (tile_base >= n) return;
    const uint32_t a = (uint32_t)st->fin_a, b = (uint32_t)st->fin_b;
    Tile t;
    tile_load(t, in, n, tile_base, a, b, s_wave);
    tile_rewrite<DELTA, false>(t, tile_sin[blockIdx.x], a, b, newid, out + tile_off[blockIdx.x], s_wsum,
                               delta, vcap, (int)min((uint64_t)TILE, n - tile_base), nullptr, nullptr);
}

}
}
// ... 1 lines not shown
```

### minbpe_amd/csrc/kernels/k_pool.hip

```cpp
#include <hip/hip_runtime.h>
#include <stdint.h>

#include "../bpe_device.h"

namespace bpe {
namespace BPE_G {

constexpr uint32_t PL_CAP = 256;
constexpr uint32_t PL_ROWS = 128;
constexpr uint32_t PL_GATHER = 1024;
static_assert(PL_GATHER >= 4 * PL_CAP, "maintain: four variants per entry");
constexpr uint32_t PL_REQ_WORDS = 2 + PL_ROWS + 256;

struct PoolScratch {
    uint32_t dl[PL_CAP];
    uint32_t rank[PL_GATHER];
    uint32_t w[8];
    uint32_t wtot[PL_CAP / 64];
    uint32_t fv, nl, k;
    uint32_t bad;
};
__device__ __forceinline__ void pool_sort(const uint32_t *ixy, const uint32_t *ic, const unsigned long long *ikey,
                                          uint32_t *oxy, uint32_t *oc, unsigned long long *okey, uint32_t n, PoolScratch &X) {
    const uint32_t tid = threadIdx.x;
    uint32_t sh = 0;
    while (sh < 4 && (n << (sh + 1)) <= blockDim.x) sh++;
    const uint32_t tpe = 1u << sh, e = tid >> sh, q = tid & (tpe - 1u);
    if (tid < n) X.rank[tid] = 0;
    __syncthreads();
    if (e < n) {
        const uint32_t c = ic[e], x = ixy[e];
        uint32_t r = 0;
#pragma unroll 4
        for (uint32_t j = q; j < n; j += tpe) {
            const uint32_t cj = ic[j];
            r += (cj > c) | ((cj == c) & (ixy[j] < x));
        }
        if (r) atomicAdd(&X.rank[e], r);
    }
    __syncthreads();
    if (tid < n) {
        const uint32_t r = X.rank[tid];
        oxy[r] = ixy[tid];
        oc[r] = ic[tid];
        okey[r] = ikey[tid];
    }
    __syncthreads();
}
constexpr int PL_KSH = 40, PL_KSH_DP = 43, PL_POS_DP = 33;
__device__ __forceinline__ void pool_level_bounds(const uint32_t *c, uint32_t n, uint32_t *ls, uint32_t *le, PoolScratch &X) {
    const uint32_t tid = threadIdx.x, w = (uint32_t)wave_id(), lane = (uint32_t)lane_id();
    const bool in = tid < n;
    const bool start = in && (tid == 0 || c[tid - 1] != c[tid]);
    const unsigned long long bal = __ballot(start);
    if (tid < PL_CAP && lane == 0) {
        X.w[w] = bal ? w * 64u + 63u - (uint32_t)__clzll((long long)bal) : 0xFFFFFFFFu;
        X.w[4 + w] = bal ? w * 64u + (uint32_t)__ffsll((long long)bal) - 1u : 0xFFFFFFFFu;
    }
    __syncthreads();
    if (in) {
        const unsigned long long upto = lane == 63 ? ~0ull : ((2ull << lane) - 1ull);
        const unsigned long long below = bal & upto, above = bal & ~upto;
        uint32_t lo = 0, hi = n;
        if (below) {
            lo = w * 64u + 63u - (uint32_t)__clzll((long long)below);
        } else {
            for (int v = (int)w - 1; v >= 0; v--)
                if (X.w[v] != 0xFFFFFFFFu) {
                    lo = X.w[v];
                    break;
                }
        }
        if (above) {
            hi = w * 64u + (uint32_t)__ffsll((long long)above) - 1u;
        } else {
            for (uint32_t v = w + 1; v < PL_CAP / 64; v++)
                if (X.w[4 + v] != 0xFFFFFFFFu) {
                    hi = X.w[4 + v];
                    break;
                }
        }
        ls[tid] = lo;
        le[tid] = hi;
    }
    __syncthreads();
}
__device__ __forceinline__ void pool_levels_dirty(const unsigned long long *key, uint32_t n, const uint32_t *ls, const uint32_t *le,
                                                  uint32_t *dirty, int ksh, PoolScratch &X) {
    const uint32_t tid = threadIdx.x;
    if (tid < n) X.dl[tid] = 0;
    __syncthreads();
    if (tid < n) {
        const uint32_t lo = ls[tid], hi = le[tid];
        const unsigned long long e0 = key[lo] >> ksh;
        if (hi - lo > 1 && (e0 == 0 || (key[tid] >> ksh) != e0)) X.dl[lo] = 1;
    }
    __syncthreads();
    if (tid < n) dirty[tid] = X.dl[ls[tid]];
    __syncthreads();
}
__device__ __forceinline__ void pool_finish(DevState *st, PoolEnt *__restrict__ pool, const uint32_t *b_xy, const uint32_t *b_c,
                                            const unsigned long long *b_key, uint32_t *a_xy, uint32_t *a_c,
                                            unsigned long long *a_key, const uint32_t *s_ls, const uint32_t *s_le,
                                            uint32_t *s_dirty, uint32_t *s_clash, uint32_t *s_k, uint32_t *s_unt, uint32_t n,
                                            uint32_t kmax, uint32_t iter, uint32_t theta, unsigned long long epoch, bool rebuilt,
                                            uint32_t hint_below, int ksh, PoolScratch &X) {
    const uint32_t tid = threadIdx.x;
    const uint32_t nwalk = min(n, kmax);
    const uint32_t sh = blockDim.x >= 4 * PL_CAP ? 2u : 0u;
    const uint32_t tpe = 1u << sh, e = tid >> sh, q = tid & (tpe - 1u);
    if (tid < n) {
        X.rank[tid] = 0;
        X.dl[tid] = 0;
    }
    if (tid == 0) {
        *s_unt = 0;
        X.bad = 0;
    }
    __syncthreads();
    if (e < n) {
        const uint32_t lo = s_ls[e], hi = s_le[e];
        const unsigned long long k = b_key[e];
        uint32_t r = 0;
#pragma unroll 4
        for (uint32_t j = lo + q; j < hi; j += tpe) {
            const unsigned long long kj = b_key[j];
            r += (kj < k) | ((kj == k) & (j < e));
        }
        if (r) atomicAdd(&X.rank[e], r);
        if (q == 0) {
            const unsigned long long e0 = b_key[lo] >> ksh;
            if (hi - lo > 1 && (e0 == 0 || (k >> ksh) != e0)) X.dl[lo] = 1;
        }
    }
    __syncthreads();
    if (tid < n) {
        const uint32_t lo = s_ls[tid];
        const uint32_t r = lo + X.rank[tid];
        a_xy[r] = b_xy[tid];
        a_c[r] = b_c[tid];
        a_key[r] = b_key[tid];
        s_dirty[r] = X.dl[lo];
    }
    __syncthreads();
    for (uint32_t q2 = tid; q2 < 32u * nwalk; q2 += blockDim.x) {
        const uint32_t i = q2 >> 5, j = q2 & 31u;
        const uint32_t x = a_xy[i] >> 16, y = a_xy[i] & 0xFFFFu;
        bool bad = false;
        if (j == i) {
            bad = (x == y) | (s_dirty[i] != 0);
        } else if (j < i) {
            const uint32_t xj = a_xy[j] >> 16, yj = a_xy[j] & 0xFFFFu;
            bad = (xj == x) | (xj == y) | (yj == x);
        }
        if (bad) atomicOr(&X.bad, 1u << i);
    }
    __syncthreads();
    if (tid == 0) *s_k = X.bad ? min(nwalk, (uint32_t)__ffs((int)X.bad) - 1u) : nwalk;
    __syncthreads();
    const uint32_t K = *s_k;
    if (tid == 0) {
        st_agent(&st->adj, 0u);
        st->count = a_c[0];
        st->ntied = s_le[0];
        st->firstpos = NOPOS;
        st->sel_tie = 0;
        st->a = (int32_t)(a_xy[0] >> 16);
        st->b = (int32_t)(a_xy[0] & 0xFFFFu);
        st->fin_a = (int32_t)(a_xy[0] >> 16);
        st->fin_b = (int32_t)(a_xy[0] & 0xFFFFu);
        st->bk = K;
        st->bz0 = 256u + iter;
        st->tl_n = st->tl_skip = 0;
        st->dp_wait = 0;
        st->sel_mode = rebuilt ? CH_FULL : CH_LIST;
        if (K == 0) {
            st->found = 0;
            st->defer = ((a_xy[0] >> 16) == (a_xy[0] & 0xFFFFu) && !s_dirty[0]) ? 1u : 2u;
            st->pool_n = 0;
            st->pool_hint_next = 1;
        } else {
            st->found = 1;
        }
    }
    if (K == 0) return;
    if (tid < K) X.rank[tid] = a_xy[tid] >> 16;
    __syncthreads();
    if (tid < 64) {
        uint32_t c = 0;
        if (tid < K) {
            c = a_c[tid];
            st->ba[tid] = (int32_t)(a_xy[tid] >> 16);
            st->bb[tid] = (int32_t)(a_xy[tid] & 0xFFFFu);
            st_agent(&st->badj[tid], 0u);
            st->bcnt[tid] = c;
        }
        const uint32_t cmax = wave_umax_dpp(c);
        const uint32_t hm = chain_hash_find(reinterpret_cast<const uint32_t *>(X.rank), K, X.rank + 256);
        if (tid == 0) {
            st->brep = cmax > CH_REP_COUNT ? (uint32_t)CH_RSTRIDE : (uint32_t)CH_REP;
            st->bhm = hm;
            st->bhm_key = ((256u + iter) << 8) | K;
        }
    }
    bool unt = false;
    if (tid >= K && tid < n) {
        PoolEnt e2;
        e2.xy = a_xy[tid];
        e2.c = a_c[tid];
        e2.key = a_key[tid];
        pool[tid - K] = e2;
        const uint32_t x = e2.xy >> 16, y = e2.xy & 0xFFFFu;
        bool touched = false;
#pragma unroll 4
        for (uint32_t p = 0; p < K; p++) touched |= ((a_xy[p] & 0xFFFFu) == x) | ((a_xy[p] >> 16) == y);
        unt = !touched;
    }
    if (tid < PL_CAP) {
        const unsigned long long ub = __ballot(unt);
        if (lane_id() == 0 && ub) atomicAdd(s_unt, (uint32_t)__popcll(ub));
    }
    __syncthreads();
    if (tid == 0) {
        st->pool_n = n - K;
        st->pool_theta = theta;
        st->pool_epoch = epoch;
        st->pool_hint_next = *s_unt < hint_below ? 1u : 0u;
    }
}

struct PoolLds {
    unsigned long long s_red[32];
    uint32_t s_words[DBITS_WORDS], s_pref[DBITS_WORDS + 1];
    uint32_t s_exrow[CH_EX_CAP], s_exm[CH_EX_CAP], s_exarg[CH_EX_CAP];
    uint32_t a_xy[PL_GATHER], a_c[PL_GATHER], b_xy[PL_GATHER], b_c[PL_GATHER];
    unsigned long long a_key[PL_GATHER], b_key[PL_GATHER];
    uint32_t s_ls[PL_CAP], s_le[PL_CAP], s_dirty[PL_CAP], s_clash[PL_CAP];
    int32_t s_tied[2 * TIE_CAP];
    unsigned long long s_pos[TIE_CAP];
    uint32_t s_lidx[TIE_CAP];
    uint32_t s_rows[PL_ROWS], s_cnt[8], s_r16[16], s_wtot[PL_CAP / 64];
    uint32_t s_fail, s_n, s_theta, s_nrows, s_nl, s_reach, s_k, s_unt, s_x;
    PoolScratch X;
    uint32_t s_sw[3 * CH_KMAX];
};
__device__ __forceinline__ void
pool_sel_body(uint32_t *__restrict__ rowmax, uint32_t *__restrict__ mat, uint32_t stride, DevState *st, const SlotRefH &ref,
              const CandArgs &C, uint32_t *__restrict__ dbits, unsigned long long *__restrict__ res, uint32_t tag,
              unsigned long long *__restrict__ req, uint32_t kcap, PoolEnt *__restrict__ pool, uint32_t *__restrict__ gather,
              uint32_t hint_below, long long *__restrict__ dpkey, unsigned long long dprank, PoolEnt *__restrict__ mid,
              PoolLds &L, const uint32_t blk, const uint32_t nblk, unsigned long long *dbg = nullptr) {
    auto dstamp = [&](int i) {
        if (dbg && threadIdx.x == 0 && blk == 0) dbg[i] = wall_clock64();
    };
    auto &s_red = L.s_red;
    auto &s_words = L.s_words;
    auto &s_pref = L.s_pref;
    auto &s_exrow = L.s_exrow;
    auto &s_exm = L.s_exm;
    auto &s_exarg = L.s_exarg;
    auto &a_xy = L.a_xy;
    auto &a_c = L.a_c;
    auto &b_xy = L.b_xy;
    auto &b_c = L.b_c;
    auto &a_key = L.a_key;
    auto &b_key = L.b_key;
    auto &s_ls = L.s_ls;
    auto &s_le = L.s_le;
    auto &s_dirty = L.s_dirty;
    auto &s_clash = L.s_clash;
    auto &s_tied = L.s_tied;
    auto &s_pos = L.s_pos;
    auto &s_lidx = L.s_lidx;
    auto &s_rows = L.s_rows;
    auto &s_cnt = L.s_cnt;
    auto &s_r16 = L.s_r16;
    auto &s_wtot = L.s_wtot;
    uint32_t &s_fail = L.s_fail, &s_n = L.s_n, &s_theta = L.s_theta, &s_nrows = L.s_nrows, &s_nl = L.s_nl, &s_k = L.s_k, &s_reach = L.s_reach,
             &s_unt = L.s_unt, &s_x = L.s_x;
    const uint32_t tid = threadIdx.x;
    enum { PW_BB = CH_KMAX, PW_STATUS = 2 * CH_KMAX, PW_DEFER, PW_GAP, PW_ITER, PW_NM, PW_HINT, PW_THETA, PW_POOLN, PW_BK, PW_BZ0, PW_EPOCH_LO, PW_EPOCH_HI, PW_N };
    PoolEnt my_ent;
    my_ent.xy = my_ent.c = 0;
    my_ent.key = 0;
    if (blk == 0 && tid < PL_CAP) my_ent = pool[tid];
    if (tid < (uint32_t)PW_N) {
        const uint32_t *base = reinterpret_cast<const uint32_t *>(st);
        uint32_t off;
        if (tid < (uint32_t)PW_BB) off = (uint32_t)offsetof(DevState, ba) / 4 + tid;
        else if (tid < (uint32_t)PW_STATUS) off = (uint32_t)offsetof(DevState, bb) / 4 + (tid - (uint32_t)PW_BB);
        else {
            static_assert(PW_N <= 3 * CH_KMAX, "s_sw");
            constexpr uint32_t o[PW_N - PW_STATUS] = {
                (uint32_t)offsetof(DevState, status) / 4,     (uint32_t)offsetof(DevState, defer) / 4,      (uint32_t)offsetof(DevState, gap) / 4,
                (uint32_t)offsetof(DevState, iter) / 4,       (uint32_t)offsetof(DevState, num_merges) / 4, (uint32_t)offsetof(DevState, pool_hint) / 4,
                (uint32_t)offsetof(DevState, pool_theta) / 4, (uint32_t)offsetof(DevState, pool_n) / 4,     (uint32_t)offsetof(DevState, bk) / 4,
                (uint32_t)offsetof(DevState, bz0) / 4,        (uint32_t)offsetof(DevState, pool_epoch) / 4, (uint32_t)offsetof(DevState, pool_epoch) / 4 + 1};
            off = o[0];
#pragma unroll
            for (int k = 1; k < PW_N - PW_STATUS; k++) off = (tid == (uint32_t)PW_STATUS + (uint32_t)k) ? o[k] : off;
        }
        L.s_sw[tid] = base[off];
    }
    __syncthreads();
    const uint32_t *s_sw = L.s_sw;
    const uint32_t status = s_sw[PW_STATUS], defer = s_sw[PW_DEFER], gap = s_sw[PW_GAP];
    const uint32_t iter = s_sw[PW_ITER], nm = s_sw[PW_NM], hint = s_sw[PW_HINT];
    if (dpkey && blk == 0 && tid < (uint32_t)DP_KEY_WORDS)
        dpkey[tid] = tid == 0 ? -(long long)status : (tid == 1 ? 0ll : 0x7FFFFFFFFFFFFFFFll);
    if (status || defer) return;
    if (iter >= nm) {
        if (blk == 0 && tid == 0) st->bk = 0;
        return;
    }
    const uint32_t vcur = 256u + iter;
    const DirtyView D{s_words, s_pref};
    if (blk != 0) {
        if (!hint) return;
        const uint32_t nd = dirty_view_build(dbits, D);
        if (nd) lean_scan_rows(mat, stride, rowmax, vcur, NOROW, NOROW, NOROW, D, 3 + nd, blk - 1, nblk - 1, res, tag,
                               true, s_red, 3);
        if (tid == 0) {
            uint32_t n = 0, th = 0;
            if (!granule_get(req, tag, n)) n = 0;
            if (n && !granule_get(req + 1 + PL_ROWS, tag, th)) n = 0;
            s_n = n;
            s_theta = th;
        }
        __syncthreads();
        const uint32_t n = s_n, theta = s_theta;
        if (blk - 1 >= n) return;
        for (uint32_t j = blk - 1; j < n; j += nblk - 1) {
            if (tid == 0) {
                uint32_t x = 0;
// ... 344 lines not shown
            for (uint32_t i = tid / PL_CAP; i < nwalk; i += blockDim.x / PL_CAP) {
                const uint32_t xi = b_xy[i] >> 16, yi = b_xy[i] & 0xFFFFu;
                if (t != i && t < s_le[i] && ((xi == x) | (xi == y) | (yi == x))) s_clash[i] = 1;
            }
            if (tid < nwalk && x == y) s_clash[tid] = 1;
        }
    }
    __syncthreads();
    if (tid < 64) {
        const unsigned long long cb = __ballot(tid < nwalk && s_clash[tid] != 0);
        const uint32_t lim = cb ? (uint32_t)__ffsll((long long)cb) - 1u : nwalk - 1u;
        if (tid == 0) s_reach = s_le[lim];
    }
    __syncthreads();
    {
        const uint32_t reach = s_reach;
        const bool locate = dpkey || (C.T != 0 && gap == 0);
        const uint32_t scan_end = min(n, reach + 48u);
        const bool cons = locate && tid < n && s_ls[tid] < scan_end && s_dirty[tid] != 0;
        const uint32_t one = cons ? 1u : 0u;
        const uint32_t inc = wave_iscan_add(one);
        if (tid < PL_CAP && lane_id() == 63) X.wtot[wave_id()] = inc;
        __syncthreads();
        uint32_t P = inc - one;
        if (tid < PL_CAP)
            for (int v = 0; v < wave_id(); v++) P += X.wtot[v];
        if (cons && s_ls[tid] == tid) {
            const uint32_t size = s_le[tid] - tid;
            if ((tid >= reach && P + size > 16u) || P + size > (uint32_t)TIE_CAP) atomicMin(&X.fv, tid);
        }
        __syncthreads();
        const bool take = cons && s_ls[tid] < X.fv;
        if (take) {
            s_tied[2 * P] = (int32_t)(b_xy[tid] >> 16);
            s_tied[2 * P + 1] = (int32_t)(b_xy[tid] & 0xFFFFu);
            s_lidx[P] = tid;
        }
        if (tid < PL_CAP) {
            const unsigned long long tb = __ballot(take);
            if (lane_id() == 0 && tb) atomicAdd(&X.nl, (uint32_t)__popcll(tb));
        }
        __syncthreads();
        if (tid == 0) s_nl = X.nl;
        __syncthreads();
    }
    const uint32_t nl = s_nl;
    dstamp(12);
    if (dpkey) {
        const bool objection = nl != 0 && gap != 0;
        if (nl && !objection) (void)tie_by_index(ref, C, s_tied, nl, s_pos);
        __syncthreads();
        if (tid == 1 && objection) dpkey[1] = -1ll;
        if (tid < nl && !objection && s_pos[tid] != NOPOS)
            dpkey[2 + tid] = (long long)((dprank << PL_POS_DP) | (s_pos[tid] & ((1ull << PL_POS_DP) - 1ull)));
        if (tid < n) {
            PoolEnt e;
            e.xy = b_xy[tid];
            e.c = b_c[tid];
            e.key = b_key[tid];
            mid[1 + tid] = e;
        }
        if (tid < nl) mid[1 + PL_CAP + tid].xy = s_lidx[tid];
        if (tid == 0) {
            PoolEnt h;
            h.xy = n | (nl << 16);
            h.c = theta;
            h.key = epoch | ((unsigned long long)(rebuilt ? 1u : 0u) << 63);
            mid[0] = h;
            st->dp_wait = 1;
            st->bk = 0;
            st->found = 0;
        }
        return;
    }
    if (nl) {
        (void)tie_by_index(ref, C, s_tied, nl, s_pos);
        __syncthreads();
        epoch++;
        if (tid < nl) b_key[s_lidx[tid]] = s_pos[tid] != NOPOS ? (epoch << PL_KSH) | s_pos[tid] : 0ull;
        __syncthreads();
    }
    dstamp(13);
    pool_finish(st, pool, b_xy, b_c, b_key, a_xy, a_c, a_key, s_ls, s_le, s_dirty, s_clash, &s_k, &s_unt, n, kmax, iter, theta,
                epoch, rebuilt, hint_below, PL_KSH, X);
    dstamp(14);
}

__global__ void __launch_bounds__(1024)
k_pool_sel(uint32_t *__restrict__ rowmax, uint32_t *__restrict__ mat, uint32_t stride, DevState *st, SlotRefH ref,
           CandArgs C, uint32_t *__restrict__ dbits, unsigned long long *__restrict__ res, uint32_t tag,
           unsigned long long *__restrict__ req, uint32_t kcap, PoolEnt *__restrict__ pool, uint32_t *__restrict__ gather,
           uint32_t hint_below, long long *__restrict__ dpkey, unsigned long long dprank, PoolEnt *__restrict__ mid) {
    __shared__ PoolLds L;
    pool_sel_body(rowmax, mat, stride, st, ref, C, dbits, res, tag, req, kcap, pool, gather, hint_below, dpkey, dprank, mid, L,
                  blockIdx.x, gridDim.x);
}

__global__ void __launch_bounds__(PL_CAP)
k_pool_sel_dp(DevState *st, const long long *__restrict__ key, uint32_t kcap, PoolEnt *__restrict__ pool,
              const PoolEnt *__restrict__ mid, uint32_t hint_below) {
    __shared__ uint32_t a_xy[PL_CAP], a_c[PL_CAP], b_xy[PL_CAP], b_c[PL_CAP];
    __shared__ unsigned long long a_key[PL_CAP], b_key[PL_CAP];
    __shared__ uint32_t s_ls[PL_CAP], s_le[PL_CAP], s_dirty[PL_CAP], s_clash[PL_CAP];
    __shared__ uint32_t s_k, s_unt;
    __shared__ PoolScratch X;
    const uint32_t tid = threadIdx.x;
    const uint32_t status = st->status;
    if (key[0] < 0 && status == 0) {
        if (tid == 0) st->status = ST_INTERNAL;
        return;
    }
    if (status || st->defer || !st->dp_wait) return;
    const PoolEnt h = mid[0];
    const uint32_t n = h.xy & 0xFFFFu, nl = h.xy >> 16, theta = h.c;
    unsigned long long epoch = h.key & 0x7FFFFFFFFFFFFFFFull;
    const bool rebuilt = (h.key >> 63) != 0;
    const uint32_t iter = st->iter, nm = st->num_merges;
    if (tid < n) {
        const PoolEnt e = mid[1 + tid];
        b_xy[tid] = e.xy;
        b_c[tid] = e.c;
        b_key[tid] = e.key;
    }
    __syncthreads();
    if (nl) {
        epoch++;
        const bool objection = key[1] < 0;
        if (tid < nl) {
            const long long p = key[2 + tid];
            b_key[mid[1 + PL_CAP + tid].xy] =
                (!objection && p != 0x7FFFFFFFFFFFFFFFll) ? (epoch << PL_KSH_DP) | (unsigned long long)p : 0ull;
        }
        __syncthreads();
    }
    pool_level_bounds(b_c, n, s_ls, s_le, X);
    pool_finish(st, pool, b_xy, b_c, b_key, a_xy, a_c, a_key, s_ls, s_le, s_dirty, s_clash, &s_k, &s_unt, n, min(kcap, nm - iter),
                iter, theta, epoch, rebuilt, hint_below, PL_KSH_DP, X);
}

}
}
```

Before: 54640 merges/s.

## Allow self-pair (a,a) merges to run on the lean chained merge path

Pool selection may now accept a self-pair (x==y) at the head of a chain, and the lean chain merge kernel gets a dedicated single-wave path for such merges. Overlapping runs of the same token need a parity carry across slot boundaries, so each wave resolves it through a decoupled lookback on per-slot descriptors. It also widens the index mask to cover the neighbouring slot. The intent is to avoid falling back to the heavier full merge/selection step whenever the top pair is (a,a). The cost is extra lookback spinning, grid size capped at the CU count on this path, and added correctness risk around run parity.

```diff
diff --git a/minbpe_amd/_native.py b/minbpe_amd/_native.py
--- a/minbpe_amd/_native.py
+++ b/minbpe_amd/_native.py
@@ -493,11 +493,11 @@
         self._check(_lib.bpe_prof_reset(self._h))
 
     def train_stats(self):
-        out = np.zeros(11, np.uint64)
-        self._check(_lib.bpe_train_stats_ex(self._h, _ptr(out), 11))
+        out = np.zeros(12, np.uint64)
+        self._check(_lib.bpe_train_stats_ex(self._h, _ptr(out), 12))
         return dict(dense=int(out[0]), sparse=int(out[1]), index_builds=int(out[2]), slots=int(out[3]),
                     lean=int(out[4]), deferred=int(out[5]), chained=int(out[6]), steps=int(out[7]),
-                    selections=int(out[8]), slot_ids=int(out[9]), fused_steps=int(out[10]))
+                    selections=int(out[8]), slot_ids=int(out[9]), fused_steps=int(out[10]), aa_in_chain=int(out[11]))
 
     def prof_read(self):
         k = len(PROF_KINDS)
diff --git a/minbpe_amd/csrc/api/api_basic.hip b/minbpe_amd/csrc/api/api_basic.hip
--- a/minbpe_amd/csrc/api/api_basic.hip
+++ b/minbpe_amd/csrc/api/api_basic.hip
@@ -193,6 +193,9 @@
     } else if (!strcmp(name, "fuse_step")) {
         if (value < 0 || value > 1) return fail(c, BPE_E_ARG, "fuse_step must be 0 or 1");
         c->fuse_step = (int)value;
+    } else if (!strcmp(name, "chain_aa")) {
+        if (value < 0 || value > 1) return fail(c, BPE_E_ARG, "chain_aa must be 0 or 1");
+        c->chain_aa = (int)value;
     } else if (!strcmp(name, "pool_hint")) {
         if (value < 0 || value > 128) return fail(c, BPE_E_ARG, "pool_hint must be 0..128");
         c->pool_hint = (int)value;
diff --git a/minbpe_amd/csrc/api/api_ctx.hip b/minbpe_amd/csrc/api/api_ctx.hip
--- a/minbpe_amd/csrc/api/api_ctx.hip
+++ b/minbpe_amd/csrc/api/api_ctx.hip
@@ -121,6 +121,8 @@
     hipEvent_t ev_stage[4] = {nullptr, nullptr, nullptr, nullptr};
     bool stage_busy[4] = {false, false, false, false};
     uint64_t n_fused = 0;
+    int chain_aa = 1;
+    uint64_t n_aa_chain = 0;
     unsigned long long *d_step_stamps = nullptr;
     int pool_hint = 0;
     PoolEnt *d_pool = nullptr;
@@ -1097,6 +1099,8 @@
     if (fused) kcap = std::min(kcap, (uint32_t)STEP_KCAP);
     const uint32_t hint_below = (uint32_t)(c->pool_hint > 0 ? c->pool_hint : (int)kcap);
     const unsigned nscan = (unsigned)std::max(1, std::min(c->chain_scan, c->num_cus - 1));
+    const bool aa_on = c->chain_aa && !fused && !c->forced && !dense && !dp && c->lean == 1 && c->idx_live && c->aa_sparse &&
+                       c->ts == TILE2_MIN && c->d_desc != nullptr;
     if (fused) {
         if (!c->d_step_pub) {
             HIPCHK(c, hipMalloc((void **)&c->d_step_pub, 64 * sizeof(unsigned long long)));
@@ -1187,7 +1191,7 @@
         hipLaunchKernelGGL(GK(c, k_pool_sel), dim3(1 + nscan), dim3(1024), 0, c->stream, c->d_rowmax, c->d_mat,
                            c->vcap, c->d_st, stream_ref_h(c), C, c->d_dbits, c->d_lean_res, ++c->lean_tag, c->d_chain_req,
                            kcap, c->d_pool, c->d_pool_gather, hint_below, dp ? c->d_dp_ckey : (long long *)nullptr,
-                           (unsigned long long)(dp ? dp->rank : 0), c->d_pool + PL_CAP);
+                           (unsigned long long)(dp ? dp->rank : 0), c->d_pool + PL_CAP, aa_on ? 1u : 0u);
     LAUNCHCHK(c, "k_pool_sel");
     if (dp) {
         TRY(dp_allreduce(c, c->d_dp_ckey, DP_KEY_WORDS, BPE_DT_INT64, BPE_OP_MIN));
@@ -1222,9 +1226,22 @@
         const unsigned g1 = std::max(1u, std::min((T + MT / 64 - 1) / (MT / 64), 5u * (unsigned)c->num_cus));
         hipLaunchKernelGGL(GK(c, k_merge_chain_dense1), dim3(g1), dim3(MT), 0, c->stream, A);
     } else {
-        const unsigned g = std::max(1u, std::min(use_index ? nwords : (T + 15) / 16, (unsigned)c->lean_grid));
+        unsigned g = std::max(1u, std::min(use_index ? nwords : (T + 15) / 16, (unsigned)c->lean_grid));
+        ChainAa X;
+        X.sdesc = c->d_desc;
+        X.removed = c->d_removed;
+        X.epoch = 0;
+        X.on = aa_on ? 1u : 0u;
+        if (aa_on) {
+            g = std::min(g, (unsigned)std::max(1, c->num_cus));
+            if ((++c->epoch & EPOCH_MASK) == 0) {
+                HIPCHK(c, hipMemsetAsync(c->d_desc, 0, ((TILE / TILE2_MIN) * c->cap_tiles + 4) * sizeof(unsigned long long), c->stream));
+                c->epoch++;
+            }
+            X.epoch = c->epoch;
+        }
         hipLaunchKernelGGL(GK(c, k_merge_chain), dim3(g), dim3(LEAN_MT), 0, c->stream, A, c->d_idx_dirty,
-                           (use_index ? 1u : 0u) | (c->chain_prefetch ? 2u : 0u), c->d_dbits);
+                           (use_index ? 1u : 0u) | (c->chain_prefetch ? 2u : 0u), c->d_dbits, X);
     }
     LAUNCHCHK(c, "k_merge_chain");
     TRY(prof_end(c));
@@ -1241,7 +1258,7 @@
     hipLaunchKernelGGL(GK(c, k_apply_chain), dim3(na + ncommit), dim3(256), 0, c->stream, c->d_mat, c->vcap, c->d_delta, dl, c->d_rowmax,
                        c->d_st, c->d_dbits, c->par, c->h_rec, c->h_srec, step, na, c->d_hdr2[c->mq], c->d_stage,
                        removed, c->d_smask, nwords, c->d_lean_sum, dp ? c->d_dp_cfold : (const uint32_t *)nullptr, fS,
-                       (const uint32_t *)ftail);
+                       (const uint32_t *)ftail, aa_on ? c->d_removed : (uint32_t *)nullptr);
     LAUNCHCHK(c, "k_apply_chain");
     TRY(prof_end(c));
     c->par ^= 1;
diff --git a/minbpe_amd/csrc/api/api_prof.hip b/minbpe_amd/csrc/api/api_prof.hip
--- a/minbpe_amd/csrc/api/api_prof.hip
+++ b/minbpe_amd/csrc/api/api_prof.hip
@@ -40,9 +40,9 @@
         TRY(read_state(c, &stt));
         chained = stt.chain_taken;
     }
-    const uint64_t v[11] = {c->n_dense, c->n_sparse, c->n_index_builds, c->slot_T, c->n_lean, c->n_deferred,
-                            chained + c->n_chained, c->n_steps, c->n_full, (uint64_t)c->ts, c->n_fused};
-    for (int i = 0; i < n && i < 11; i++) out[i] = v[i];
+    const uint64_t v[12] = {c->n_dense, c->n_sparse, c->n_index_builds, c->slot_T, c->n_lean, c->n_deferred,
+                            chained + c->n_chained, c->n_steps, c->n_full, (uint64_t)c->ts, c->n_fused, c->n_aa_chain};
+    for (int i = 0; i < n && i < 12; i++) out[i] = v[i];
     return BPE_OK;
 }
 
diff --git a/minbpe_amd/csrc/api/api_rccl.hip b/minbpe_amd/csrc/api/api_rccl.hip
--- a/minbpe_amd/csrc/api/api_rccl.hip
+++ b/minbpe_amd/csrc/api/api_rccl.hip
@@ -120,6 +120,7 @@
     int general_until = -1, defer_hold = 0, defer_strikes = 0;
     uint64_t lean_at_last_defer = 0, n_chain_merges = 0;
     c->n_lean = c->n_deferred = 0;
+    c->n_aa_chain = 0;
     c->n_steps = c->n_full = c->n_chained = 0;
     c->rows_pending = false;
     c->sum_valid = false;
diff --git a/minbpe_amd/csrc/api/api_train.hip b/minbpe_amd/csrc/api/api_train.hip
--- a/minbpe_amd/csrc/api/api_train.hip
+++ b/minbpe_amd/csrc/api/api_train.hip
@@ -58,6 +58,7 @@
     c->n_lean = c->n_deferred = 0;
     c->n_steps = c->n_full = c->n_chained = 0;
     c->n_fused = 0;
+    c->n_aa_chain = 0;
     static const char *stamp_path = getenv("BPE_STEP_STAMPS");
     const size_t stamp_bytes = (size_t)STEP_STAMP_RING * (3 * 16 + 256 * 2) * sizeof(unsigned long long);
     if (stamp_path) {
@@ -321,6 +322,7 @@
                     for (uint32_t j = 0; j < sr.k && !stop; j++) {
                         TRY(wait_iter((int)(sr.first_iter + j)));
                         TRY(take_record((int)(sr.first_iter + j), true));
+                        if (!stop && c->h_rec[sr.first_iter + j].a == c->h_rec[sr.first_iter + j].b) c->n_aa_chain++;
                     }
                     if (sr.k) {
                         c->n_lean += sr.k;
diff --git a/minbpe_amd/csrc/bpe_device.h b/minbpe_amd/csrc/bpe_device.h
--- a/minbpe_amd/csrc/bpe_device.h
+++ b/minbpe_amd/csrc/bpe_device.h
@@ -186,6 +186,12 @@
     uint32_t *idx;
     uint32_t istride;
 };
+struct ChainAa {
+    unsigned long long *sdesc;
+    uint32_t *removed;
+    uint32_t epoch;
+    uint32_t on;
+};
 struct PoolEnt {
     uint32_t xy, c;
     unsigned long long key;
diff --git a/minbpe_amd/csrc/kernels/k_chain.hip b/minbpe_amd/csrc/kernels/k_chain.hip
--- a/minbpe_amd/csrc/kernels/k_chain.hip
+++ b/minbpe_amd/csrc/kernels/k_chain.hip
@@ -317,6 +317,149 @@
     }
 }
 
+__device__ __forceinline__ void merge_aa_wave(uint32_t *scr, const uint32_t t, const AbArgs &A, const ChainAa &X, const uint32_t a,
+                                              const uint32_t newid, const uint32_t Tl) {
+    const int lane = lane_id();
+    uint32_t *s_hdr = scr, *s_halo = scr + 8;
+    uint4 hv6 = (lane & 1) ? make_uint4(INVALID_WORD, INVALID_WORD, 0u, 0u) : make_uint4(INVALID_WORD, INVALID_WORD, INVALID_WORD, 0u);
+    {
+        const long long hi = 2ll * (long long)t - 2 + lane;
+        if (lane < 6 && hi >= 0 && hi < 2ll * (long long)A.T) hv6 = reinterpret_cast<const uint4 *>(A.hdr_in)[hi];
+    }
+    const uint32_t mi = bcast(hv6.w, 2);
+    const int len = (int)(mi & 0x7FFFFFFFu);
+    if (len == 0) return;
+    const uint32_t cur = mi >> 31;
+    const uint32_t *src = (cur ? A.b1 : A.b0) + (size_t)t * TILE2;
+    const uint32_t first = bcast(hv6.x, 2);
+    uint32_t halo0 = bcast(hv6.x, 4), halo1 = bcast(hv6.y, 4), halo2 = bcast(hv6.z, 4);
+    uint32_t prev1 = bcast(hv6.y, 1);
+    uint32_t tnext = t + 1;
+    {
+        const uint32_t nlen = bcast(hv6.w, 4) & 0x7FFFFFFFu, plen = bcast(hv6.w, 0) & 0x7FFFFFFFu;
+        if ((t + 1 < Tl && nlen < 3) || (t > 0 && plen < 2)) {
+            uint32_t ctx[7] = {0, 0, 0, 0, 0, 0, 0};
+            if (lane == 0) slot_context_walk(A.hdr_in, t, Tl, ctx);
+            halo0 = bcast(ctx[0], 0);
+            halo1 = bcast(ctx[1], 0);
+            halo2 = bcast(ctx[2], 0);
+            prev1 = bcast(ctx[4], 0);
+            tnext = bcast(ctx[6], 0);
+        }
+    }
+    const uint32_t hw1 = bcast(hv6.y, 2), hw2 = bcast(hv6.z, 2), hl0 = bcast(hv6.x, 3), hl1 = bcast(hv6.y, 3);
+    if (lane == 0) {
+        s_hdr[0] = first;
+        s_hdr[1] = hw1;
+        s_hdr[2] = hw2;
+        s_hdr[3] = mi;
+        s_hdr[4] = hl0;
+        s_hdr[5] = hl1;
+        s_halo[0] = halo0;
+        s_halo[1] = halo1;
+        s_halo[2] = halo2;
+    }
+    SlotRaw raw;
+    slot_raw_load<true>(raw, src, len);
+    __builtin_amdgcn_fence(__ATOMIC_RELEASE, "wavefront");
+    __builtin_amdgcn_wave_barrier();
+    __builtin_amdgcn_fence(__ATOMIC_ACQUIRE, "wavefront");
+    Tile tl;
+    tile_from_slot<true>(tl, raw, len, s_halo);
+    tile_rbits(tl, a, a);
+    uint32_t s = (uint32_t)((prev1 != INVALID_WORD) & ((prev1 & IDMASK) == a) & ((first & NWMASK) == a));
+    {
+        const unsigned long long tag = ((unsigned long long)(X.epoch & EPOCH_MASK)) << 42;
+        uint32_t sc = 0;
+        bool failed = false;
+        if (s) {
+            uint32_t u = t;
+            uint32_t mu = 0;
+            while (u-- > 0) {
+                mu = A.hdr_in[u].meta;
+                if (mu & 0x7FFFFFFFu) break;
+            }
+            const int lu = (int)(mu & 0x7FFFFFFFu);
+            const uint32_t *pu = ((mu >> 31) ? A.b1 : A.b0) + (size_t)u * TILE2;
+            int ones = 0;
+            bool open = true;
+            uint32_t nextw = first;
+            for (int base = lu - 1; base >= 0 && open; base -= 64) {
+                const int q = base - lane;
+                const uint32_t xq = (q >= 0) ? pu[q] : INVALID_WORD;
+                uint32_t nx = (uint32_t)__shfl_up((int)xq, 1);
+                if (lane == 0) nx = nextw;
+                const bool r = (q >= 0) && ((xq & IDMASK) == a) && ((nx & NWMASK) == a);
+                const unsigned long long zeros = __ballot(!r);
+                if (zeros) {
+                    ones += __ffsll((long long)zeros) - 1;
+                    const int zl = __ffsll((long long)zeros) - 1;
+                    open = (base - zl < 0);
+                    break;
+                }
+                ones += 64;
+                nextw = (uint32_t)__shfl((int)xq, 63);
+            }
+            if (!open || ones < lu) {
+                sc = (uint32_t)(ones & 1);
+            } else {
+                uint32_t su = 0;
+                bool got = false;
+                for (uint32_t spins = 0; spins < LOOKBACK_SPINS; spins++) {
+                    const unsigned long long d = desc_load(&X.sdesc[u]);
+                    if ((d >> 42) == (tag >> 42) + (1ull << 20)) {
+                        su = (uint32_t)(d & 1u);
+                        got = true;
+                        break;
+                    }
+                    __builtin_amdgcn_s_sleep(8);
+                }
+                failed = !got;
+                sc = (uint32_t)(((lu - 1) & 1) == 0) ^ su;
+            }
+        }
+        if (lane == 0) {
+            desc_store(&X.sdesc[t], tag | (1ull << 62) | sc);
+            if (failed) atomicExch(&A.st->status, ST_LOOKBACK);
+        }
+        s = sc;
+    }
+    {
+        uint32_t anyr = s;
+        const int q0 = lane * 4;
+        const int nb = len + 1 - q0;
+        const uint32_t keep = nb >= 4 ? 0xFu : (nb <= 0 ? 0u : ((1u << nb) - 1u));
+        anyr |= tl.rb[0] & keep;
+        if (len == TILE2) anyr |= (uint32_t)(((tl.tail[0] & IDMASK) == a) & ((tl.tail[1] & NWMASK) == a));
+        if (!__any(anyr != 0)) return;
+    }
+    tile_lzscan<true>(tl, nullptr);
+    uint32_t kept = 0;
+    bool changed = false;
+    uint32_t *dst = (cur ? A.b0 : A.b1) + (size_t)t * TILE2;
+    tile_rewrite<true, true, 1, true>(tl, s, a, a, newid, dst, nullptr, A.delta, A.vcap, len, &kept, &changed, s_hdr, A.idx,
+                                      A.istride, t, tnext, t);
+    __builtin_amdgcn_fence(__ATOMIC_RELEASE, "wavefront");
+    __builtin_amdgcn_wave_barrier();
+    __builtin_amdgcn_fence(__ATOMIC_ACQUIRE, "wavefront");
+    if (lane == 0 && changed) {
+        uint32_t h[8];
+        h[0] = kept > 0 ? s_hdr[0] : INVALID_WORD;
+        h[1] = kept > 1 ? s_hdr[1] : INVALID_WORD;
+        h[2] = kept > 2 ? s_hdr[2] : INVALID_WORD;
+        h[3] = kept | ((cur ^ 1u) << 31);
+        h[4] = kept > 1 ? s_hdr[4] : INVALID_WORD;
+        h[5] = kept > 0 ? s_hdr[5] : INVALID_WORD;
+        h[6] = h[7] = 0;
+        stage_put<false>(A.stage + t, t, h);
+        atomicOr(&A.smask[t >> 5], 1u << (t & 31));
+        atomicAdd(&X.removed[(t & 255u) * REMOVED_STRIDE], (uint32_t)len - kept);
+        if (kept < 3 && t + 1 < Tl) A.st->gap = 1;
+    }
+    __builtin_amdgcn_fence(__ATOMIC_RELEASE, "wavefront");
+    __builtin_amdgcn_wave_barrier();
+}
+
 __device__ __forceinline__ uint32_t chain_hash_find(const uint32_t *pa, uint32_t K, uint32_t *tab) {
     if (K < 5) return 0u;
     const uint32_t lane = (uint32_t)lane_id(), half = lane >> 5, l = lane & 31u;
@@ -370,7 +513,7 @@
                                                  MergeLds &L, const uint32_t K, const uint32_t z0, const uint32_t brep,
                                                  const uint32_t blk, const uint32_t nblk, unsigned long long *dbg = nullptr,
                                                  const bool have_st = false, const uint32_t tlive_in = 0, const uint32_t gap_in = 0,
-                                                 const bool pre_ok = false, const uint32_t pre_hm = 0) {
+                                                 const bool pre_ok = false, const uint32_t pre_hm = 0, const ChainAa *X = nullptr) {
     auto dstamp = [&](int i) {
         if (dbg && threadIdx.x == 0) dbg[i] = wall_clock64();
     };
@@ -389,7 +532,14 @@
     AbArgs A1 = A;
     A1.newid = z0;
     const uint32_t a0 = s_pa[0], b0 = s_pb[0];
+    const bool aa = MJ == 1 && X != nullptr && X->on && K == 1 && a0 == b0;
     auto do_slot = [&](uint32_t t) {
+        if constexpr (MJ == 1) {
+            if (aa) {
+                merge_aa_wave(s_out[wave_id()], t, A, *X, a0, z0, Tl);
+                return;
+            }
+        }
         if (K == 1) {
             merge_ab_wave<true, true, false, THROUGH>(s_out[wave_id()], nullptr, t, A1, a0, b0, Tl);
         } else {
@@ -417,6 +567,16 @@
                 pair_hash(s_pa[p], s_pb[p], h1, h2, h3);
                 mk |= A.idx[(size_t)h1 * A.istride + w] & A.idx[(size_t)h2 * A.istride + w] &
                       A.idx[(size_t)h3 * A.istride + w];
+            }
+            if (aa) {
+                uint32_t nx = 0;
+                if (w + 1 < nwords) {
+                    uint32_t h1, h2, h3;
+                    pair_hash(a0, a0, h1, h2, h3);
+                    nx = idx_dirty[w + 1] | (A.idx[(size_t)h1 * A.istride + w + 1] & A.idx[(size_t)h2 * A.istride + w + 1] &
+                                             A.idx[(size_t)h3 * A.istride + w + 1]);
+                }
+                mk |= (mk >> 1) | (nx << 31);
             }
             const uint32_t left = Tl - w * 32;
             if (left < 32) mk &= (1u << left) - 1u;
@@ -481,7 +641,7 @@
     __syncthreads();
 }
 __global__ void __launch_bounds__(LEAN_MT)
-k_merge_chain(AbArgs A, const uint32_t *__restrict__ idx_dirty, uint32_t use_index, uint32_t *__restrict__ dbits) {
+k_merge_chain(AbArgs A, const uint32_t *__restrict__ idx_dirty, uint32_t use_index, uint32_t *__restrict__ dbits, ChainAa X) {
     __shared__ MergeLds L;
     __shared__ uint32_t s_w[SW_WORDS];
     DevState *st = A.st;
@@ -502,8 +662,12 @@
         if (threadIdx.x == 0) L.s_pb1[0] = 0xFFFFFFFFu;
     }
     __syncthreads();
+    if (K == 1 && s_w[0] == s_w[SW_BB] && !(MJ == 1 && X.on)) {
+        if (blockIdx.x == 0 && threadIdx.x == 0) atomicExch(&st->status, ST_INTERNAL);
+        return;
+    }
     merge_chain_body(A, idx_dirty, use_index, L, K, z0, brep, blockIdx.x, gridDim.x, nullptr, true, s_w[SW_TLIVE], s_w[SW_GAP],
-                     s_w[SW_BHM_KEY] == ((z0 << 8) | K), s_w[SW_BHM]);
+                     s_w[SW_BHM_KEY] == ((z0 << 8) | K), s_w[SW_BHM], &X);
 }
 
 constexpr int CH_KDENSE = 6;
@@ -611,7 +775,36 @@
             rm = reinterpret_cast<const uint2 *>(rowmax)[t];
         }
         bool flagged = false;
-        if (K == 1) {
+        if (!OWNED && K == 1 && pair_a(0) == pair_b(0)) {
+            const uint32_t a = pair_a(0), Z = z0;
+            constexpr int RB = 4;
+            uint32_t acc[4] = {0, 0, 0, 0};
+            const uint32_t old_ta = live ? mat[(size_t)t * stride + a] : 0u;
+            for (uint32_t r0 = 0; r0 < nrep; r0 += RB) {
+                uint32_t x[RB][4];
+#pragma unroll
+                for (int k = 0; k < RB; k++)
+#pragma unroll
+                    for (int v = 0; v < 4; v++)
+                        x[k][v] = (live && r0 + k < nrep) ? delta[delta_rep_off(r0 + k, vc) + (size_t)v * vc + t] : 0u;
+#pragma unroll
+                for (int k = 0; k < RB; k++)
+#pragma unroll
+                    for (int v = 0; v < 4; v++) {
+                        if (x[k][v]) delta[delta_rep_off(r0 + k, vc) + (size_t)v * vc + t] = 0;
+                        acc[v] += x[k][v];
+                    }
+            }
+            if (acc[0]) {
+                atomicSub(&mat[(size_t)t * stride + a], acc[0]);
+                flagged |= old_ta == rm.x;
+            }
+            if (acc[1]) atomicSub(&mat[(size_t)a * stride + t], acc[1]);
+            if (acc[2]) atomicAdd(&mat[(size_t)t * stride + Z], acc[2]);
+            if (acc[3]) atomicAdd(&mat[(size_t)Z * stride + t], acc[3]);
+            if (live && t == a) mat[(size_t)a * stride + a] = 0;
+            flagged |= live && ((t == a) | (t == Z));
+        } else if (K == 1) {
             const uint32_t a = pair_a(0), b = pair_b(0), Z = z0;
             const uint32_t adj = folded ? ftail[0] : adjs[0];
             constexpr int RB = OWNED ? 8 : 16;
@@ -742,8 +935,10 @@
 }
 __device__ __forceinline__ void apply_chain_records(DevState *st, int par, IterRec *rec, StepRec *srec, uint32_t step,
                                                     uint32_t *__restrict__ removed, const uint32_t K, const bool noop,
-                                                    const uint32_t status, const uint32_t defer, const uint32_t remote) {
+                                                    const uint32_t status, const uint32_t defer, const uint32_t remote,
+                                                    uint32_t *__restrict__ removed_aa = nullptr) {
     {
+        if (removed_aa && !noop && K == 1 && st->ba[0] == st->bb[0]) removed = removed_aa;
         uint32_t v = 0;
         if (removed) {
 #pragma unroll
@@ -823,7 +1018,8 @@
               const uint32_t *__restrict__ rowmax, DevState *st, uint32_t *__restrict__ dbits, int par, IterRec *rec,
               StepRec *srec, uint32_t step, uint32_t na, SlotHdr *__restrict__ hdr_cur, const StageRec *__restrict__ stage,
               uint32_t *__restrict__ removed, uint32_t *__restrict__ smask, uint32_t nwords, uint4 *__restrict__ sums,
-              const uint32_t *__restrict__ folded, uint32_t fS, const uint32_t *__restrict__ ftail) {
+              const uint32_t *__restrict__ folded, uint32_t fS, const uint32_t *__restrict__ ftail,
+              uint32_t *__restrict__ removed_aa) {
     __shared__ uint32_t s_w[SW_WORDS], s_pairs[CH_KMAX];
     step_words_fetch(st, s_w);
     const uint32_t remote = (folded && ftail[16] != 0) ? 1u : 0u;
@@ -839,7 +1035,7 @@
                                   ftail, K, z0, 0u, s_pairs, s_w + SW_BADJ, s_w[SW_BREP]);
         return;
     }
-    if (blockIdx.x == na && threadIdx.x < 64) apply_chain_records(st, par, rec, srec, step, removed, K, noop, status, defer, remote);
+    if (blockIdx.x == na && threadIdx.x < 64) apply_chain_records(st, par, rec, srec, step, removed, K, noop, status, defer, remote, removed_aa);
     if (noop) return;
     apply_chain_commit((blockIdx.x - na) * blockDim.x + threadIdx.x, (gridDim.x - na) * blockDim.x, nwords, smask, stage, hdr_cur);
 }
diff --git a/minbpe_amd/csrc/kernels/k_merge.hip b/minbpe_amd/csrc/kernels/k_merge.hip
--- a/minbpe_amd/csrc/kernels/k_merge.hip
+++ b/minbpe_amd/csrc/kernels/k_merge.hip
@@ -36,8 +36,9 @@
     uint4 v[MJ];
     uint32_t tail[3];
 };
+template <bool W1 = false>
 __device__ __forceinline__ void slot_raw_load(SlotRaw &r, const uint32_t *__restrict__ src, int len) {
-    const int lane = lane_id(), wrel = wave_id() * WAVE_SPAN;
+    const int lane = lane_id(), wrel = W1 ? 0 : wave_id() * WAVE_SPAN;
 #pragma unroll
     for (int j = 0; j < MJ; j++) {
         const int q0 = wrel + j * 256 + lane * 4;
@@ -50,8 +51,9 @@
         r.tail[i] = (q < len) ? src[q] : 0u;
     }
 }
+template <bool W1 = false>
 __device__ __forceinline__ void tile_from_slot(Tile &t, const SlotRaw &r, int len, const uint32_t *halo) {
-    const int lane = lane_id(), wrel = wave_id() * WAVE_SPAN;
+    const int lane = lane_id(), wrel = W1 ? 0 : wave_id() * WAVE_SPAN;
 #pragma unroll
     for (int j = 0; j < MJ; j++) {
         const int q0 = wrel + j * 256 + lane * 4;
@@ -88,8 +90,9 @@
         t.rb[j] = rb;
     }
 }
+template <bool W1 = false>
 __device__ __forceinline__ void tile_lzscan(Tile &t, int *s_wave) {
-    const int lane = lane_id(), wave = wave_id();
+    const int lane = lane_id(), wave = W1 ? 0 : wave_id();
     int lzg[MJ];
     const int gb0 = wave * WAVE_SPAN + lane * 4;
 #pragma unroll
@@ -105,6 +108,7 @@
         t.E[j] = max(carry, ex);
         carry = max(carry, (int)lane_last((uint32_t)v));
     }
+    if (W1) return;
     if (lane == 0) s_wave[wave] = carry;
     __syncthreads();
     int win = -1;
@@ -127,8 +131,9 @@
     return (uint32_t)((q - lz) & 1) ^ ((lz < 0) ? s : 0u);
 }
 
+template <bool W1 = false>
 __device__ __forceinline__ uint32_t group_mbits(const Tile &t, int j, uint32_t s, uint32_t &mprev) {
-    const int q0 = wave_id() * WAVE_SPAN + j * 256 + lane_id() * 4;
+    const int q0 = (W1 ? 0 : wave_id() * WAVE_SPAN) + j * 256 + lane_id() * 4;
     int lz = t.E[j];
     mprev = (q0 == 0) ? s : ((lz == q0 - 1) ? 0u : parity_bit(q0 - 1, lz, s));
     uint32_t mb = 0;
@@ -457,21 +462,22 @@
     }
 }
 
-template <bool DELTA, bool SKIP_UNCHANGED, int HL = 0>
+template <bool DELTA, bool SKIP_UNCHANGED, int HL = 0, bool W1 = false>
 __device__ __forceinline__ void tile_rewrite(const Tile &t, uint32_t s, uint32_t a, uint32_t b,
                                              uint32_t newid, uint32_t *__restrict__ dst_tile,
                                              uint32_t *s_wsum, uint32_t *__restrict__ delta,
                                              uint32_t vcap, int own_len, uint32_t *kept_out,
                                              bool *changed_out, uint32_t *__restrict__ hdr4 = nullptr,
                                              uint32_t *__restrict__ idx = nullptr, uint32_t istride = 0,
-                                             uint32_t tself = 0, uint32_t tnext = 0xFFFFFFFFu) {
-    const int lane = lane_id(), wave = wave_id();
+                                             uint32_t tself = 0, uint32_t tnext = 0xFFFFFFFFu,
+                                             uint32_t rep_sel = 0xFFFFFFFFu) {
+    const int lane = lane_id(), wave = W1 ? 0 : wave_id();
     uint32_t mb[MJ], mp[MJ], kb[MJ], ex[MJ];
     uint32_t carry = 0, chg = 0;
     const int qw = wave * WAVE_SPAN + lane * 4;
 #pragma unroll
     for (int j = 0; j < MJ; j++) {
-        mb[j] = group_mbits(t, j, s, mp[j]);
+        mb[j] = group_mbits<W1>(t, j, s, mp[j]);
         uint32_t valid = 0;
 #pragma unroll
         for (int k = 0; k < 4; k++) valid |= (uint32_t)(qw + j * 256 + k < own_len) << k;
@@ -482,15 +488,20 @@
         carry += lane_last(v);
     }
     const bool wchg = __any(chg != 0);
-    if (lane == 0) s_wsum[wave] = carry | (wchg ? 0x80000000u : 0u);
-    __syncthreads();
     uint32_t wbase = 0, total = 0;
     bool changed = (s != 0);
-    for (int w = 0; w < MT / 64; w++) {
-        const uint32_t v = s_wsum[w];
-        if (w < wave) wbase += v & 0x7FFFFFFFu;
-        total += v & 0x7FFFFFFFu;
-        changed |= (v >> 31) != 0;
+    if (W1) {
+        total = carry;
+        changed |= wchg;
+    } else {
+        if (lane == 0) s_wsum[wave] = carry | (wchg ? 0x80000000u : 0u);
+        __syncthreads();
+        for (int w = 0; w < MT / 64; w++) {
+            const uint32_t v = s_wsum[w];
+            if (w < wave) wbase += v & 0x7FFFFFFFu;
+            total += v & 0x7FFFFFFFu;
+            changed |= (v >> 31) != 0;
+        }
     }
     if (kept_out) *kept_out = total;
     if (changed_out) *changed_out = changed;
@@ -542,7 +553,7 @@
         if (!__any(near != 0)) return;
         const uint32_t nrep = 1u << (vcap >> 24);
         vcap &= 0xFFFFFFu;
-        delta += delta_rep_off(blockIdx.x & (nrep - 1), vcap);
+        delta += delta_rep_off((rep_sel != 0xFFFFFFFFu ? rep_sel : blockIdx.x) & (nrep - 1), vcap);
 #pragma unroll
         for (int j = 0; j < MJ; j++) {
             const uint32_t nb_m = lane_next(mb[j], 0);
diff --git a/minbpe_amd/csrc/kernels/k_pool.hip b/minbpe_amd/csrc/kernels/k_pool.hip
--- a/minbpe_amd/csrc/kernels/k_pool.hip
+++ b/minbpe_amd/csrc/kernels/k_pool.hip
@@ -104,7 +104,7 @@
                                             unsigned long long *a_key, const uint32_t *s_ls, const uint32_t *s_le,
                                             uint32_t *s_dirty, uint32_t *s_clash, uint32_t *s_k, uint32_t *s_unt, uint32_t n,
                                             uint32_t kmax, uint32_t iter, uint32_t theta, unsigned long long epoch, bool rebuilt,
-                                            uint32_t hint_below, int ksh, PoolScratch &X) {
+                                            uint32_t hint_below, int ksh, PoolScratch &X, const bool aa_ok = false) {
     const uint32_t tid = threadIdx.x;
     const uint32_t nwalk = min(n, kmax);
     const uint32_t sh = blockDim.x >= 4 * PL_CAP ? 2u : 0u;
@@ -148,10 +148,11 @@
         const uint32_t x = a_xy[i] >> 16, y = a_xy[i] & 0xFFFFu;
         bool bad = false;
         if (j == i) {
-            bad = (x == y) | (s_dirty[i] != 0);
+            bad = ((x == y) & !(aa_ok && i == 0)) | (s_dirty[i] != 0);
         } else if (j < i) {
             const uint32_t xj = a_xy[j] >> 16, yj = a_xy[j] & 0xFFFFu;
-            bad = (xj == x) | (xj == y) | (yj == x);
+            if (j == 0 && xj == yj) bad = true;
+            bad |= (xj == x) | (xj == y) | (yj == x);
         }
         if (bad) atomicOr(&X.bad, 1u << i);
     }
@@ -203,13 +204,14 @@
             st->bhm_key = ((256u + iter) << 8) | K;
         }
     }
+    const uint32_t Kout = (K == 1 && (a_xy[0] >> 16) == (a_xy[0] & 0xFFFFu)) ? 0u : K;
     bool unt = false;
-    if (tid >= K && tid < n) {
+    if (tid >= Kout && tid < n) {
         PoolEnt e2;
         e2.xy = a_xy[tid];
         e2.c = a_c[tid];
         e2.key = a_key[tid];
-        pool[tid - K] = e2;
+        pool[tid - Kout] = e2;
         const uint32_t x = e2.xy >> 16, y = e2.xy & 0xFFFFu;
         bool touched = false;
 #pragma unroll 4
@@ -222,7 +224,7 @@
     }
     __syncthreads();
     if (tid == 0) {
-        st->pool_n = n - K;
+        st->pool_n = n - Kout;
         st->pool_theta = theta;
         st->pool_epoch = epoch;
         st->pool_hint_next = *s_unt < hint_below ? 1u : 0u;
@@ -249,7 +251,7 @@
               const CandArgs &C, uint32_t *__restrict__ dbits, unsigned long long *__restrict__ res, uint32_t tag,
               unsigned long long *__restrict__ req, uint32_t kcap, PoolEnt *__restrict__ pool, uint32_t *__restrict__ gather,
               uint32_t hint_below, long long *__restrict__ dpkey, unsigned long long dprank, PoolEnt *__restrict__ mid,
-              PoolLds &L, const uint32_t blk, const uint32_t nblk, unsigned long long *dbg = nullptr) {
+              PoolLds &L, const uint32_t blk, const uint32_t nblk, unsigned long long *dbg = nullptr, const bool aa_ok = false) {
     auto dstamp = [&](int i) {
         if (dbg && threadIdx.x == 0 && blk == 0) dbg[i] = wall_clock64();
     };
@@ -760,7 +762,7 @@
     }
     dstamp(13);
     pool_finish(st, pool, b_xy, b_c, b_key, a_xy, a_c, a_key, s_ls, s_le, s_dirty, s_clash, &s_k, &s_unt, n, kmax, iter, theta,
-                epoch, rebuilt, hint_below, PL_KSH, X);
+                epoch, rebuilt, hint_below, PL_KSH, X, aa_ok);
     dstamp(14);
 }
 
@@ -768,10 +770,11 @@
 k_pool_sel(uint32_t *__restrict__ rowmax, uint32_t *__restrict__ mat, uint32_t stride, DevState *st, SlotRefH ref,
            CandArgs C, uint32_t *__restrict__ dbits, unsigned long long *__restrict__ res, uint32_t tag,
            unsigned long long *__restrict__ req, uint32_t kcap, PoolEnt *__restrict__ pool, uint32_t *__restrict__ gather,
-           uint32_t hint_below, long long *__restrict__ dpkey, unsigned long long dprank, PoolEnt *__restrict__ mid) {
+           uint32_t hint_below, long long *__restrict__ dpkey, unsigned long long dprank, PoolEnt *__restrict__ mid,
+           uint32_t aa_ok) {
     __shared__ PoolLds L;
     pool_sel_body(rowmax, mat, stride, st, ref, C, dbits, res, tag, req, kcap, pool, gather, hint_below, dpkey, dprank, mid, L,
-                  blockIdx.x, gridDim.x);
+                  blockIdx.x, gridDim.x, nullptr, aa_ok != 0);
 }
 
 __global__ void __launch_bounds__(PL_CAP)
```

Measured after the change: 56380 merges/s (median of 6 runs). 1.03x the previous value.
